# Muennighoff/sgpt

Hardware: AMD Instinct MI355X
Metric: encoded sentences/sec (SGPT-125M, seq_len 128, encode + weighted-mean pool + cosine top-10 chunk loop) (higher is better)
Workload: dtype f16

## Files before the change

### include/sgpt_hip.h

```cpp
#ifndef SGPT_HIP_H
#define SGPT_HIP_H

#include <stddef.h>
#include <stdint.h>

#ifdef __cplusplus
extern "C" {
#endif

#define SGPT_ABI_VERSION 21

typedef int sgpt_status;
#define SGPT_OK 0
#define SGPT_ERR_INVALID (-1)
#define SGPT_ERR_HIP (-2)
#define SGPT_ERR_MISSING (-3)
#define SGPT_ERR_OOM (-4)
#define SGPT_ERR_COMM (-6)
#define SGPT_ERR_RANGE (-5)

typedef struct sgpt_ctx sgpt_ctx;
typedef struct sgpt_model sgpt_model;

enum { SGPT_F32 = 0, SGPT_BF16 = 1, SGPT_FP8W = 2, SGPT_F16 = 3, SGPT_FP8M = 4 };
enum { SGPT_ARCH_GPTNEO = 0, SGPT_ARCH_GPTJ = 1, SGPT_ARCH_BLOOM = 2, SGPT_ARCH_BERT = 3, SGPT_ARCH_LLAMA = 4 };
enum { SGPT_POOL_WEIGHTEDMEAN = 0, SGPT_POOL_MEAN = 1, SGPT_POOL_LASTTOKEN = 2, SGPT_POOL_LEARNTMEAN = 3,
       SGPT_POOL_CLS = 4 };
enum { SGPT_COS = 0, SGPT_DOT = 1, SGPT_NEG_L2 = 2 };

typedef struct {
    int32_t arch;
    int32_t n_layers;
    int32_t d_model;
    int32_t n_heads;
    int32_t d_ffn;
    int32_t vocab;
    int32_t max_pos;
    int32_t window;
    float ln_eps;
    float attn_scale;
    int32_t compute_dtype;
    const uint8_t* layer_is_local;
    int32_t rotary_dim;
    int32_t qk_split;
    int32_t split_weights;
    int32_t n_kv_heads;
} sgpt_model_desc;

typedef struct {
    const char* name;
    const float* ptr;
    int64_t numel;
} sgpt_tensor_view;

int sgpt_abi_version(void);
sgpt_status sgpt_ctx_create(int hip_device, sgpt_ctx** out);
void sgpt_ctx_destroy(sgpt_ctx* ctx);
const char* sgpt_last_error(const sgpt_ctx* ctx);

sgpt_status sgpt_model_load(sgpt_ctx* ctx, const sgpt_model_desc* desc,
                            const sgpt_tensor_view* tensors, size_t n_tensors, sgpt_model** out);
void sgpt_model_free(sgpt_model* model);

sgpt_status sgpt_model_calibrate_begin(sgpt_model* model);
sgpt_status sgpt_model_calibrate_end(sgpt_model* model, float margin, float* scales_out);
sgpt_status sgpt_model_set_act_scales(sgpt_model* model, const float* scales, int32_t n_scales);

sgpt_status sgpt_encode(sgpt_model* model, const int32_t* ids, const int32_t* pos,
                        const int32_t* seq_off, const int32_t* seq_len, const int32_t* pad_left,
                        int32_t B, int32_t T_pad, int32_t max_alloc_len,
                        int32_t pool_mode, int32_t n_layers_run, int32_t apply_final_ln,
                        int32_t normalize, float* out, float* hidden_out, void* stream);

sgpt_status sgpt_encode_layers(sgpt_model* model, const int32_t* ids, const int32_t* pos,
                               const int32_t* seq_off, const int32_t* seq_len, const int32_t* pad_left,
                               int32_t B, int32_t T_pad, int32_t max_alloc_len, int32_t pool_mode,
                               int32_t normalize, float* out_layers, float* out_mean, void* stream);

sgpt_status sgpt_model_set_pool_weights(sgpt_model* model, const float* weights, int32_t n);

sgpt_status sgpt_lm_logprobs(sgpt_model* model, const float* hidden, const int32_t* row_idx, const int32_t* targets,
                             int32_t n, float* out_logprob, int32_t* out_greedy, void* stream);

sgpt_status sgpt_pool(sgpt_ctx* ctx, const void* hidden, int32_t hidden_dtype, const int32_t* mask,
                      int32_t B, int32_t S, int32_t d, int32_t pool_mode, float* out, void* stream);
sgpt_status sgpt_pool_learnt(sgpt_ctx* ctx, const void* hidden, int32_t hidden_dtype, const int32_t* mask,
                             int32_t B, int32_t S, int32_t d, const float* pos_weights, float* out, void* stream);

sgpt_status sgpt_l2_normalize(sgpt_ctx* ctx, const float* in, int64_t n, int32_t d,
                              void* out, int32_t out_dtype, void* stream);

sgpt_status sgpt_pairwise_scores(sgpt_ctx* ctx, const float* a, const float* b, int64_t n, int32_t d, int32_t cosine,
                                 float* out, void* stream);

sgpt_status sgpt_f32_to_16(sgpt_ctx* ctx, const float* in, int64_t numel, void* out, int32_t out_dtype, void* stream);
sgpt_status sgpt_f32_to_bf16(sgpt_ctx* ctx, const float* in, int64_t numel, void* out, void* stream);

sgpt_status sgpt_model_range_check(sgpt_model* model, int32_t* flagged, int32_t reset, void* stream);
sgpt_status sgpt_model_range_adapt(sgpt_model* model, int32_t* n_raised, void* stream);
sgpt_status sgpt_model_get_range_shifts(sgpt_model* model, int32_t* shifts, int32_t n);
sgpt_status sgpt_model_set_range_shifts(sgpt_model* model, const int32_t* shifts, int32_t n);
sgpt_status sgpt_range_check(sgpt_ctx* ctx, int32_t* flagged, int32_t reset, void* stream);

#define SGPT_PREC_CLASSES 5
enum { SGPT_PC_LN1 = 0, SGPT_PC_ATT = 1, SGPT_PC_CTX = 2, SGPT_PC_LN2 = 3, SGPT_PC_H = 4 };
sgpt_status sgpt_model_set_precision(sgpt_model* model, const int32_t* plan, int32_t n);
sgpt_status sgpt_model_get_precision(sgpt_model* model, int32_t* plan, int32_t n);
sgpt_status sgpt_model_release_split_weights(sgpt_model* model, int64_t* bytes_freed);
sgpt_status sgpt_model_precision_probe_begin(sgpt_model* model);
sgpt_status sgpt_model_precision_probe_end(sgpt_model* model, float* crest_out );
sgpt_status sgpt_row_crest(sgpt_ctx* ctx, const void* x, int32_t dtype, int64_t n, int32_t d, int64_t ld, float* crest_out,
                           void* stream);
sgpt_status sgpt_split16(sgpt_ctx* ctx, const float* in, int64_t n, int32_t d, int32_t layout, void* out, int32_t out_dtype,
                         void* stream);
sgpt_status sgpt_linear_split(sgpt_ctx* ctx, int32_t dtype, int32_t epi, const void* A, const void* W, const float* bias,
                              void* out, int64_t ldo, int64_t lo_delta, int64_t hi2_delta, int32_t M, int32_t N, int32_t K,
                              void* stream);

uint64_t sgpt_ctx_generation(const sgpt_ctx* ctx);
sgpt_status sgpt_ctx_reserve(sgpt_ctx* ctx, size_t encode_bytes, size_t score_bytes);

sgpt_status sgpt_fp8_quantize_rows(sgpt_ctx* ctx, const float* w, int64_t rows, int64_t cols,
                                   uint8_t* codes, float* scale, void* stream);
sgpt_status sgpt_fp8_dequantize_rows(sgpt_ctx* ctx, const uint8_t* codes, const float* scale, int64_t rows,
                                     int64_t cols, void* out, int32_t out_dtype, void* stream);

sgpt_status sgpt_scores(sgpt_ctx* ctx, const void* a, const void* b, int32_t dtype,
                        int64_t na, int64_t nb, int32_t d, float* out, int64_t ldo, void* stream);

sgpt_status sgpt_score_topk(sgpt_ctx* ctx, const void* q, const void* corpus, int32_t dtype,
                            int32_t nq, int64_t N, int32_t d, int32_t k, int64_t idx_base,
                            float* run_val, int64_t* run_idx, int32_t n_run, int32_t* n_out,
                            void* stream);

sgpt_status sgpt_score_topk_q8(sgpt_ctx* ctx, const void* q, const uint8_t* codes, const float* scale, int32_t nq, int64_t N, int32_t d,
                               int32_t k, int64_t idx_base, float* run_val, int64_t* run_idx, int32_t n_run, int32_t* n_out,
                               void* stream);

sgpt_status sgpt_pack_sign_bits(sgpt_ctx* ctx, const float* x, int64_t n, int32_t d, const float* center ,
                                uint8_t* bits, int64_t ldb, void* stream);

sgpt_status sgpt_score_topk_bits(sgpt_ctx* ctx, const float* q, const uint8_t* bits, int64_t ldb, int32_t nq, int64_t N, int32_t d,
                                 int32_t k, int32_t kp, int32_t mode, const uint8_t* codes, const float* scale, int64_t idx_base,
                                 float* run_val, int64_t* run_idx, int32_t n_run, int32_t* n_out, void* stream);

sgpt_status sgpt_u8_col_minmax(sgpt_ctx* ctx, const float* x, int64_t n, int32_t d, int32_t accumulate, float* col_min, float* col_max,
                               void* stream);
sgpt_status sgpt_u8_quantize_rows(sgpt_ctx* ctx, const float* x, int64_t n, int32_t d, int32_t ld, const float* start, const float* step,
                                  uint8_t* codes, void* stream);
sgpt_status sgpt_u8_dequantize_rows(sgpt_ctx* ctx, const uint8_t* codes, int64_t n, int32_t ld, const float* start, const float* step,
                                    void* out, int32_t out_dtype, void* stream);

sgpt_status sgpt_u8_prepare_queries(sgpt_ctx* ctx, const float* q, const float* start, const float* step, int32_t nq, int32_t d, int32_t ld,
                                    void* qpad, float* qscale, float* qbias, void* stream);

sgpt_status sgpt_score_topk_u8(sgpt_ctx* ctx, const float* q, const uint8_t* codes, const float* start, const float* step, int32_t nq,
                               int64_t N, int32_t d, int32_t ld, int32_t k, int64_t idx_base, float* run_val, int64_t* run_idx,
                               int32_t n_run, int32_t* n_out, void* stream);

sgpt_status sgpt_u8_rescore(sgpt_ctx* ctx, const float* q, const uint8_t* codes, const float* start, const float* step, int32_t nq, int64_t N,
                            int32_t d, int32_t ld, const int64_t* idx, int64_t ld_idx, int32_t m, int64_t idx_base, float* out_val,
                            int64_t* out_idx, void* stream);

sgpt_status sgpt_score_topk_bits_u8(sgpt_ctx* ctx, const float* q, const float* center , const uint8_t* bits, int64_t ldb,
                                    const uint8_t* codes, const float* start, const float* step, int32_t ld, int32_t nq, int64_t N, int32_t d,
                                    int32_t k, int32_t kp, int64_t idx_base, float* run_val, int64_t* run_idx, int32_t n_run, int32_t* n_out,
                                    void* stream);

sgpt_status sgpt_score_overflow_count(sgpt_ctx* ctx, int32_t* n_chunks, int32_t* n_overflowed, void* stream);

sgpt_status sgpt_score_topk_refined(sgpt_ctx* ctx, const float* q, const float* corpus32, const void* corpus16, int32_t dtype16,
                                    int32_t nq, int64_t N, int32_t d, int32_t k, int64_t idx_base, float margin,
                                    float* run_val, int64_t* run_idx, int32_t n_run, int32_t* n_out, int32_t* fallback_flag_out,
                                    void* stream);

sgpt_status sgpt_topk_merge(sgpt_ctx* ctx, const float* val, const int64_t* idx, int32_t nq,
                            int32_t m, int32_t k, const int64_t* exclude_idx,
                            float* out_val, int64_t* out_idx, void* stream);

#define SGPT_COMM_ID_BYTES 128
sgpt_status sgpt_comm_unique_id(uint8_t* id );
sgpt_status sgpt_comm_init(sgpt_ctx* ctx, const uint8_t* id, int32_t rank, int32_t world);
sgpt_status sgpt_comm_destroy(sgpt_ctx* ctx);
int32_t sgpt_comm_world(const sgpt_ctx* ctx);
int32_t sgpt_comm_rank(const sgpt_ctx* ctx);
sgpt_status sgpt_allgather_rows(sgpt_ctx* ctx, const void* local, const int64_t* counts, int64_t row_bytes, void* out,
                                void* stream);
sgpt_status sgpt_allgather_rows_padded(sgpt_ctx* ctx, const void* local, const int64_t* counts, int64_t row_bytes, void* out,
                                       void* stream);
sgpt_status sgpt_exchange_topk(sgpt_ctx* ctx, const float* val, const int64_t* idx, int32_t nq, int32_t k, int32_t k_out,
                               const int64_t* exclude_idx, float* out_val, int64_t* out_idx, void* stream);
sgpt_status sgpt_fold_gathered_topk(sgpt_ctx* ctx, const float* gathered_val, const int64_t* gathered_idx, int32_t world,
                                    int32_t nq, int32_t k, int32_t k_out, const int64_t* exclude_idx, float* out_val,
                                    int64_t* out_idx, void* stream);

sgpt_status sgpt_topk(sgpt_ctx* ctx, const float* scores, int32_t nq, int64_t n, int64_t ld,
                      int32_t k, int64_t idx_base, float* out_val, int64_t* out_idx, void* stream);

#define SGPT_EVAL_MAX_CUTS 16
sgpt_status sgpt_eval_ranked(sgpt_ctx* ctx, const int64_t* idx, const float* val, int32_t nq, int32_t K,
                             const int32_t* qrel_off, const int64_t* qrel_pos, const int32_t* qrel_rel,
                             const int32_t* ideal_rel, const int32_t* k_values, int32_t nk, int32_t check_order,
                             int32_t* out_hits, int32_t* out_first, float* out_dcg, float* out_idcg, float* out_sp,
                             int32_t* out_R, void* stream);

#define SGPT_EVAL_MAX_GROUP 1024
sgpt_status sgpt_eval_groups(sgpt_ctx* ctx, const float* emb, int32_t n_rows, int32_t d, int32_t mode, const float* scores_in,
                             int32_t G, const int32_t* grp_off, int32_t n_cand, int32_t max_group, const int32_t* q_row,
                             const int32_t* cand_row, const int32_t* cand_rel, const int32_t* R_extra,
                             const int32_t* ideal_off, const int32_t* ideal_rel, int32_t n_ideal, float* out_scores,
                             int32_t* out_order, int32_t* out_hits1, int32_t* out_hits5, int32_t* out_first, int32_t* out_R, float* out_sp,
                             float* out_dcg, float* out_idcg, void* stream);

#define SGPT_EVAL_MAX_PAIRS (1 << 24)
sgpt_status sgpt_eval_pairs(sgpt_ctx* ctx, const float* score, const int32_t* label, int32_t n, int32_t check_nan,
                            int32_t* out_rank2, int64_t* out_n_pos, int64_t* out_n_used, double* out_ap_num, void* stream);

sgpt_status sgpt_linear(sgpt_ctx* ctx, int32_t dtype, int32_t epi, int32_t out_dtype, const void* A, const void* W,
                        const float* bias, const float* resid, void* out, int32_t M, int32_t N, int32_t K, void* stream);

sgpt_status sgpt_linear_query(sgpt_ctx* ctx, int32_t dtype, int32_t epi, const void* A, const float* x, const float* ln_gamma,
                              const float* ln_beta, float ln_eps, const void* W, const float* bias, const float* resid, void* out,
                              void* out_vt, int32_t n_split, int32_t M, int32_t N, int32_t K, void* stream);

sgpt_status sgpt_linear_qkv(sgpt_ctx* ctx, int32_t dtype, const void* A, const void* W, void* out, void* out_vt, int32_t n_split,
                            int32_t M, int32_t N, int32_t K, void* stream);

sgpt_status sgpt_attention(sgpt_ctx* ctx, int32_t dtype, const void* q, const void* k, const void* v, int64_t ldq, int64_t ldvt,
                           void* out, int64_t ldo, const int32_t* seq_off, int32_t B, int32_t T, int32_t H, int32_t dh,
                           int32_t window, float scale, const float* alibi, int32_t max_alloc_len, int32_t out_fp8,
                           float out_scale, int32_t* range_flag, int32_t x3, int64_t qk_lo_delta, int64_t v_lo_delta,
                           int64_t ctx_lo_delta, int64_t ctx_hi2_delta, void* stream);

sgpt_status sgpt_attention_ex(sgpt_ctx* ctx, int32_t dtype, const void* q, const void* k, const void* v, int64_t ldq, int64_t ldvt,
                              void* out, int64_t ldo, const int32_t* seq_off, int32_t B, int32_t T, int32_t H, int32_t dh,
                              int32_t window, float scale, const float* alibi, int32_t max_alloc_len, int32_t out_fp8,
                              float out_scale, int32_t* range_flag, int32_t x3, int64_t qk_lo_delta, int64_t v_lo_delta,
                              int64_t ctx_lo_delta, int64_t ctx_hi2_delta, int32_t causal, const int32_t* seq_len, void* stream);

sgpt_status sgpt_attention_gqa(sgpt_ctx* ctx, int32_t dtype, const void* q, const void* k, const void* v, int64_t ldq, int64_t ldvt,
                               void* out, int64_t ldo, const int32_t* seq_off, int32_t B, int32_t T, int32_t H, int32_t n_kv_heads,
                               int32_t dh, int32_t window, float scale, const float* alibi, int32_t max_alloc_len, int32_t out_fp8,
                               float out_scale, int32_t* range_flag, int32_t x3, int64_t qk_lo_delta, int64_t v_lo_delta,
                               int64_t ctx_lo_delta, int64_t ctx_hi2_delta, void* stream);

sgpt_status sgpt_embed(sgpt_ctx* ctx, const int32_t* ids, const int32_t* pos, const float* wte, const float* wpe, int32_t T,
                       int32_t d, int32_t vocab, int32_t max_pos, float* out, void* stream);
sgpt_status sgpt_layernorm(sgpt_ctx* ctx, const float* x, const float* gamma, const float* beta, int32_t T, int32_t d, float eps,
                           void* out, int32_t out_dtype, float out_mul, int32_t split, void* stream);
sgpt_status sgpt_layernorm_writeback(sgpt_ctx* ctx, float* x, const float* gamma, const float* beta, int32_t T, int32_t d, float eps,
                                     void* out16, int32_t out_dtype, void* stream);
sgpt_status sgpt_rmsnorm(sgpt_ctx* ctx, const float* x, const float* gamma, int32_t T, int32_t d, float eps, void* out, int32_t out_dtype,
                         void* stream);
sgpt_status sgpt_swiglu(sgpt_ctx* ctx, const void* gu, int32_t dtype, int32_t T, int32_t ffn, void* out, void* stream);
sgpt_status sgpt_rope_half(sgpt_ctx* ctx, void* buf, int32_t dtype, int64_t ld, int64_t k_off, const int32_t* pos, const float* sin_t,
                           const float* cos_t, int32_t T, int32_t H, int32_t H_kv, int32_t head_dim, int32_t max_pos, void* stream);
sgpt_status sgpt_qknorm_rope_half(sgpt_ctx* ctx, void* buf, int32_t dtype, int64_t ld, int64_t k_off, const int32_t* pos,
                                  const float* sin_t, const float* cos_t, int32_t T, int32_t H, int32_t H_kv, int32_t head_dim,
                                  int32_t max_pos, const float* q_gamma, const float* k_gamma, float eps, void* stream);
sgpt_status sgpt_lnf_pool_ex(sgpt_ctx* ctx, const float* x, const float* gamma, const float* beta, const int32_t* seq_off,
                             const int32_t* seq_len, const int32_t* pad_left, int32_t B, int32_t d, float eps, int32_t apply_ln,
                             int32_t mode, int32_t normalize, const float* pos_weights, int32_t n_weights, float* out,
                             int32_t* nonfinite_flag, int32_t norm_kind, void* stream);
sgpt_status sgpt_lnf_pool(sgpt_ctx* ctx, const float* x, const float* gamma, const float* beta, const int32_t* seq_off,
                          const int32_t* seq_len, const int32_t* pad_left, int32_t B, int32_t d, float eps, int32_t apply_ln,
                          int32_t mode, int32_t normalize, const float* pos_weights, int32_t n_weights, float* out,
                          int32_t* nonfinite_flag, void* stream);
sgpt_status sgpt_rope(sgpt_ctx* ctx, void* buf, int32_t dtype, int64_t ld, int64_t k_off, const int32_t* pos, const float* sin,
                      const float* cos, int32_t T, int32_t H, int32_t head_dim, int32_t rotary_dim, int32_t max_pos, void* stream);
sgpt_status sgpt_logprob_rows(sgpt_ctx* ctx, const float* logits, int64_t ld, int32_t V, const int32_t* targets, int32_t n,
                              float* out_logprob, int32_t* out_greedy, void* stream);

sgpt_status sgpt_layernorm_fp8(sgpt_ctx* ctx, const float* x, const float* gamma, const float* beta, int32_t T, int32_t d,
                               float eps, uint8_t* codes, float* row_scale, void* stream);
sgpt_status sgpt_linear_fp8(sgpt_ctx* ctx, int32_t epi, int32_t out_dtype, const uint8_t* A, const float* a_scale,
                            float a_scalar, const uint8_t* W, const float* w_scale, const float* bias, const float* resid,
                            void* out, float out_scale, int32_t M, int32_t N, int32_t K, void* stream);

sgpt_status sgpt_prof_enable(sgpt_ctx* ctx, int32_t on);
sgpt_status sgpt_prof_read(sgpt_ctx* ctx, int64_t* launches, double* ms, double* flops, int32_t reset);

int32_t sgpt_ctx_set_gemm_cu_cap(sgpt_ctx* ctx, int32_t n);
int32_t sgpt_ctx_set_low_latency(sgpt_ctx* ctx, int32_t on);
int32_t sgpt_ctx_set_tile_policy(sgpt_ctx* ctx, int32_t policy);
int32_t sgpt_ctx_set_query_tile(sgpt_ctx* ctx, int32_t k);

sgpt_status sgpt_bench_gemm(sgpt_ctx* ctx, int32_t dtype, int32_t epi, int32_t out_dtype,
                            int32_t M, int32_t N, int32_t K, int32_t iters, float* ms_out);

#ifdef __cplusplus
}
#endif
#endif
```

### sgpt_amd/_lib.py

```python
import ctypes as C
import os

HERE = os.path.dirname(os.path.abspath(__file__))
LIB_PATH = os.environ.get("SGPT_HIP_LIB") or os.path.join(HERE, "lib", "libsgpt_hip.so")

SGPT_F32, SGPT_BF16, SGPT_FP8W, SGPT_F16, SGPT_FP8M = 0, 1, 2, 3, 4
SGPT_ABI_VERSION = 21
SGPT_PREC_CLASSES = 5
PC_LN1, PC_ATT, PC_CTX, PC_LN2, PC_H = 0, 1, 2, 3, 4
SGPT_ERR_RANGE = -5
SGPT_ERR_COMM = -6
SGPT_COMM_ID_BYTES = 128
SGPT_EVAL_MAX_CUTS = 16
SGPT_EVAL_MAX_GROUP = 1024
SGPT_EVAL_MAX_PAIRS = 1 << 24
SGPT_COS, SGPT_DOT, SGPT_NEG_L2 = 0, 1, 2
SGPT_ARCH_GPTNEO, SGPT_ARCH_GPTJ, SGPT_ARCH_BLOOM, SGPT_ARCH_BERT, SGPT_ARCH_LLAMA = 0, 1, 2, 3, 4
POOL_MODES = {"weightedmean": 0, "mean": 1, "lasttoken": 2, "learntmean": 3, "cls": 4}
EPI_BIAS_GELU_ERF = 9


class ModelDesc(C.Structure):
    _fields_ = [("arch", C.c_int32), ("n_layers", C.c_int32), ("d_model", C.c_int32), ("n_heads", C.c_int32),
                ("d_ffn", C.c_int32), ("vocab", C.c_int32), ("max_pos", C.c_int32), ("window", C.c_int32),
                ("ln_eps", C.c_float), ("attn_scale", C.c_float), ("compute_dtype", C.c_int32),
                ("layer_is_local", C.POINTER(C.c_uint8)), ("rotary_dim", C.c_int32), ("qk_split", C.c_int32),
                ("split_weights", C.c_int32), ("n_kv_heads", C.c_int32)]


class TensorView(C.Structure):
    _fields_ = [("name", C.c_char_p), ("ptr", C.c_void_p), ("numel", C.c_int64)]


SIGNATURES = {
    "sgpt_abi_version": (C.c_int, []),
    "sgpt_ctx_create": (C.c_int, [C.c_int, C.POINTER(C.c_void_p)]),
    "sgpt_ctx_destroy": (None, [C.c_void_p]),
    "sgpt_last_error": (C.c_char_p, [C.c_void_p]),
    "sgpt_model_load": (C.c_int, [C.c_void_p, C.POINTER(ModelDesc), C.POINTER(TensorView), C.c_size_t,
                                  C.POINTER(C.c_void_p)]),
    "sgpt_model_free": (None, [C.c_void_p]),
    "sgpt_encode": (C.c_int, [C.c_void_p, C.c_void_p, C.c_void_p, C.c_void_p, C.c_void_p, C.c_void_p,
                              C.c_int32, C.c_int32, C.c_int32, C.c_int32, C.c_int32, C.c_int32, C.c_int32,
                              C.c_void_p, C.c_void_p, C.c_void_p]),
    "sgpt_encode_layers": (C.c_int, [C.c_void_p, C.c_void_p, C.c_void_p, C.c_void_p, C.c_void_p, C.c_void_p,
                                     C.c_int32, C.c_int32, C.c_int32, C.c_int32, C.c_int32, C.c_void_p, C.c_void_p,
                                     C.c_void_p]),
    "sgpt_model_set_pool_weights": (C.c_int, [C.c_void_p, C.c_void_p, C.c_int32]),
    "sgpt_pool_learnt": (C.c_int, [C.c_void_p, C.c_void_p, C.c_int32, C.c_void_p, C.c_int32, C.c_int32, C.c_int32,
                                   C.c_void_p, C.c_void_p, C.c_void_p]),
    "sgpt_fp8_quantize_rows": (C.c_int, [C.c_void_p, C.c_void_p, C.c_int64, C.c_int64, C.c_void_p, C.c_void_p,
                                         C.c_void_p]),
    "sgpt_fp8_dequantize_rows": (C.c_int, [C.c_void_p, C.c_void_p, C.c_void_p, C.c_int64, C.c_int64, C.c_void_p,
                                           C.c_int32, C.c_void_p]),
    "sgpt_lm_logprobs": (C.c_int, [C.c_void_p, C.c_void_p, C.c_void_p, C.c_void_p, C.c_int32, C.c_void_p, C.c_void_p,
                                   C.c_void_p]),
    "sgpt_pool": (C.c_int, [C.c_void_p, C.c_void_p, C.c_int32, C.c_void_p, C.c_int32, C.c_int32, C.c_int32,
                            C.c_int32, C.c_void_p, C.c_void_p]),
    "sgpt_l2_normalize": (C.c_int, [C.c_void_p, C.c_void_p, C.c_int64, C.c_int32, C.c_void_p, C.c_int32, C.c_void_p]),
    "sgpt_pairwise_scores": (C.c_int, [C.c_void_p, C.c_void_p, C.c_void_p, C.c_int64, C.c_int32, C.c_int32, C.c_void_p, C.c_void_p]),
    "sgpt_f32_to_bf16": (C.c_int, [C.c_void_p, C.c_void_p, C.c_int64, C.c_void_p, C.c_void_p]),
    "sgpt_f32_to_16": (C.c_int, [C.c_void_p, C.c_void_p, C.c_int64, C.c_void_p, C.c_int32, C.c_void_p]),
    "sgpt_range_check": (C.c_int, [C.c_void_p, C.POINTER(C.c_int32), C.c_int32, C.c_void_p]),
    "sgpt_ctx_generation": (C.c_uint64, [C.c_void_p]),
    "sgpt_ctx_reserve": (C.c_int, [C.c_void_p, C.c_size_t, C.c_size_t]),
    "sgpt_scores": (C.c_int, [C.c_void_p, C.c_void_p, C.c_void_p, C.c_int32, C.c_int64, C.c_int64, C.c_int32,
                              C.c_void_p, C.c_int64, C.c_void_p]),
    "sgpt_score_topk": (C.c_int, [C.c_void_p, C.c_void_p, C.c_void_p, C.c_int32, C.c_int32, C.c_int64, C.c_int32,
                                  C.c_int32, C.c_int64, C.c_void_p, C.c_void_p, C.c_int32, C.POINTER(C.c_int32),
                                  C.c_void_p]),
    "sgpt_score_topk_q8": (C.c_int, [C.c_void_p, C.c_void_p, C.c_void_p, C.c_void_p, C.c_int32, C.c_int64, C.c_int32,
                                     C.c_int32, C.c_int64, C.c_void_p, C.c_void_p, C.c_int32, C.POINTER(C.c_int32),
                                     C.c_void_p]),
    "sgpt_score_topk_u8": (C.c_int, [C.c_void_p, C.c_void_p, C.c_void_p, C.c_void_p, C.c_void_p, C.c_int32, C.c_int64, C.c_int32, C.c_int32,
                                     C.c_int32, C.c_int64, C.c_void_p, C.c_void_p, C.c_int32, C.POINTER(C.c_int32), C.c_void_p]),
    "sgpt_u8_col_minmax": (C.c_int, [C.c_void_p, C.c_void_p, C.c_int64, C.c_int32, C.c_int32, C.c_void_p, C.c_void_p, C.c_void_p]),
    "sgpt_u8_quantize_rows": (C.c_int, [C.c_void_p, C.c_void_p, C.c_int64, C.c_int32, C.c_int32, C.c_void_p, C.c_void_p, C.c_void_p,
                                        C.c_void_p]),
    "sgpt_u8_dequantize_rows": (C.c_int, [C.c_void_p, C.c_void_p, C.c_int64, C.c_int32, C.c_void_p, C.c_void_p, C.c_void_p, C.c_int32,
                                          C.c_void_p]),
    "sgpt_u8_prepare_queries": (C.c_int, [C.c_void_p, C.c_void_p, C.c_void_p, C.c_void_p, C.c_int32, C.c_int32, C.c_int32, C.c_void_p,
                                          C.c_void_p, C.c_void_p, C.c_void_p]),
    "sgpt_pack_sign_bits": (C.c_int, [C.c_void_p, C.c_void_p, C.c_int64, C.c_int32, C.c_void_p, C.c_void_p, C.c_int64, C.c_void_p]),
    "sgpt_score_topk_bits": (C.c_int, [C.c_void_p, C.c_void_p, C.c_void_p, C.c_int64, C.c_int32, C.c_int64, C.c_int32, C.c_int32,
                                       C.c_int32, C.c_int32, C.c_void_p, C.c_void_p, C.c_int64, C.c_void_p, C.c_void_p, C.c_int32,
                                       C.POINTER(C.c_int32), C.c_void_p]),
    "sgpt_u8_rescore": (C.c_int, [C.c_void_p, C.c_void_p, C.c_void_p, C.c_void_p, C.c_void_p, C.c_int32, C.c_int64, C.c_int32, C.c_int32,
                                  C.c_void_p, C.c_int64, C.c_int32, C.c_int64, C.c_void_p, C.c_void_p, C.c_void_p]),
    "sgpt_score_topk_bits_u8": (C.c_int, [C.c_void_p, C.c_void_p, C.c_void_p, C.c_void_p, C.c_int64, C.c_void_p, C.c_void_p, C.c_void_p,
                                          C.c_int32, C.c_int32, C.c_int64, C.c_int32, C.c_int32, C.c_int32, C.c_int64, C.c_void_p,
                                          C.c_void_p, C.c_int32, C.POINTER(C.c_int32), C.c_void_p]),
    "sgpt_score_overflow_count": (C.c_int, [C.c_void_p, C.POINTER(C.c_int32), C.POINTER(C.c_int32), C.c_void_p]),
    "sgpt_score_topk_refined": (C.c_int, [C.c_void_p, C.c_void_p, C.c_void_p, C.c_void_p, C.c_int32, C.c_int32, C.c_int64, C.c_int32,
                                           C.c_int32, C.c_int64, C.c_float, C.c_void_p, C.c_void_p, C.c_int32, C.c_void_p, C.c_void_p,
                                           C.c_void_p]),
    "sgpt_topk_merge": (C.c_int, [C.c_void_p, C.c_void_p, C.c_void_p, C.c_int32, C.c_int32, C.c_int32, C.c_void_p,
                                  C.c_void_p, C.c_void_p, C.c_void_p]),
    "sgpt_topk": (C.c_int, [C.c_void_p, C.c_void_p, C.c_int32, C.c_int64, C.c_int64, C.c_int32, C.c_int64,
                            C.c_void_p, C.c_void_p, C.c_void_p]),
    "sgpt_eval_ranked": (C.c_int, [C.c_void_p, C.c_void_p, C.c_void_p, C.c_int32, C.c_int32, C.c_void_p, C.c_void_p, C.c_void_p,
                                   C.c_void_p, C.POINTER(C.c_int32), C.c_int32, C.c_int32, C.c_void_p, C.c_void_p, C.c_void_p,
                                   C.c_void_p, C.c_void_p, C.c_void_p, C.c_void_p]),
    "sgpt_eval_groups": (C.c_int, [C.c_void_p, C.c_void_p, C.c_int32, C.c_int32, C.c_int32, C.c_void_p, C.c_int32, C.c_void_p, C.c_int32,
                                   C.c_int32, C.c_void_p, C.c_void_p, C.c_void_p, C.c_void_p, C.c_void_p, C.c_void_p, C.c_int32,
                                   C.c_void_p, C.c_void_p, C.c_void_p, C.c_void_p, C.c_void_p, C.c_void_p, C.c_void_p, C.c_void_p,
                                   C.c_void_p, C.c_void_p]),
    "sgpt_eval_pairs": (C.c_int, [C.c_void_p, C.c_void_p, C.c_void_p, C.c_int32, C.c_int32, C.c_void_p, C.c_void_p, C.c_void_p,
                                  C.c_void_p, C.c_void_p]),
    "sgpt_linear": (C.c_int, [C.c_void_p, C.c_int32, C.c_int32, C.c_int32, C.c_void_p, C.c_void_p, C.c_void_p, C.c_void_p,
                              C.c_void_p, C.c_int32, C.c_int32, C.c_int32, C.c_void_p]),
    "sgpt_linear_query": (C.c_int, [C.c_void_p, C.c_int32, C.c_int32, C.c_void_p, C.c_void_p, C.c_void_p, C.c_void_p, C.c_float, C.c_void_p,
                                    C.c_void_p, C.c_void_p, C.c_void_p, C.c_void_p, C.c_int32, C.c_int32, C.c_int32, C.c_int32, C.c_void_p]),
    "sgpt_linear_qkv": (C.c_int, [C.c_void_p, C.c_int32, C.c_void_p, C.c_void_p, C.c_void_p, C.c_void_p, C.c_int32, C.c_int32, C.c_int32,
                                  C.c_int32, C.c_void_p]),
    "sgpt_model_calibrate_begin": (C.c_int, [C.c_void_p]),
    "sgpt_model_calibrate_end": (C.c_int, [C.c_void_p, C.c_float, C.c_void_p]),
    "sgpt_model_set_act_scales": (C.c_int, [C.c_void_p, C.c_void_p, C.c_int32]),
    "sgpt_layernorm_fp8": (C.c_int, [C.c_void_p, C.c_void_p, C.c_void_p, C.c_void_p, C.c_int32, C.c_int32, C.c_float, C.c_void_p,
                                     C.c_void_p, C.c_void_p]),
    "sgpt_linear_fp8": (C.c_int, [C.c_void_p, C.c_int32, C.c_int32, C.c_void_p, C.c_void_p, C.c_float, C.c_void_p, C.c_void_p,
                                  C.c_void_p, C.c_void_p, C.c_void_p, C.c_float, C.c_int32, C.c_int32, C.c_int32, C.c_void_p]),
    "sgpt_comm_unique_id": (C.c_int, [C.c_void_p]),
    "sgpt_comm_init": (C.c_int, [C.c_void_p, C.c_void_p, C.c_int32, C.c_int32]),
    "sgpt_comm_destroy": (C.c_int, [C.c_void_p]),
    "sgpt_comm_world": (C.c_int32, [C.c_void_p]),
    "sgpt_comm_rank": (C.c_int32, [C.c_void_p]),
    "sgpt_allgather_rows": (C.c_int, [C.c_void_p, C.c_void_p, C.c_void_p, C.c_int64, C.c_void_p, C.c_void_p]),
    "sgpt_allgather_rows_padded": (C.c_int, [C.c_void_p, C.c_void_p, C.c_void_p, C.c_int64, C.c_void_p, C.c_void_p]),
    "sgpt_exchange_topk": (C.c_int, [C.c_void_p, C.c_void_p, C.c_void_p, C.c_int32, C.c_int32, C.c_int32, C.c_void_p,
                                     C.c_void_p, C.c_void_p, C.c_void_p]),
    "sgpt_fold_gathered_topk": (C.c_int, [C.c_void_p, C.c_void_p, C.c_void_p, C.c_int32, C.c_int32, C.c_int32, C.c_int32,
                                          C.c_void_p, C.c_void_p, C.c_void_p, C.c_void_p]),
    "sgpt_ctx_set_low_latency": (C.c_int32, [C.c_void_p, C.c_int32]),
    "sgpt_ctx_set_tile_policy": (C.c_int32, [C.c_void_p, C.c_int32]),
    "sgpt_ctx_set_gemm_cu_cap": (C.c_int32, [C.c_void_p, C.c_int32]),
    "sgpt_ctx_set_query_tile": (C.c_int32, [C.c_void_p, C.c_int32]),
    "sgpt_model_range_check": (C.c_int, [C.c_void_p, C.POINTER(C.c_int32), C.c_int32, C.c_void_p]),
    "sgpt_model_range_adapt": (C.c_int, [C.c_void_p, C.POINTER(C.c_int32), C.c_void_p]),
    "sgpt_model_get_range_shifts": (C.c_int, [C.c_void_p, C.c_void_p, C.c_int32]),
    "sgpt_model_set_range_shifts": (C.c_int, [C.c_void_p, C.c_void_p, C.c_int32]),
    "sgpt_model_set_precision": (C.c_int, [C.c_void_p, C.c_void_p, C.c_int32]),
    "sgpt_model_get_precision": (C.c_int, [C.c_void_p, C.c_void_p, C.c_int32]),
    "sgpt_model_release_split_weights": (C.c_int, [C.c_void_p, C.c_void_p]),
    "sgpt_model_precision_probe_begin": (C.c_int, [C.c_void_p]),
    "sgpt_model_precision_probe_end": (C.c_int, [C.c_void_p, C.c_void_p]),
    "sgpt_row_crest": (C.c_int, [C.c_void_p, C.c_void_p, C.c_int32, C.c_int64, C.c_int32, C.c_int64, C.POINTER(C.c_float), C.c_void_p]),
    "sgpt_split16": (C.c_int, [C.c_void_p, C.c_void_p, C.c_int64, C.c_int32, C.c_int32, C.c_void_p, C.c_int32, C.c_void_p]),
    "sgpt_linear_split": (C.c_int, [C.c_void_p, C.c_int32, C.c_int32, C.c_void_p, C.c_void_p, C.c_void_p, C.c_void_p,
                                    C.c_int64, C.c_int64, C.c_int64, C.c_int32, C.c_int32, C.c_int32, C.c_void_p]),
    "sgpt_attention": (C.c_int, [C.c_void_p, C.c_int32, C.c_void_p, C.c_void_p, C.c_void_p, C.c_int64, C.c_int64,
                                 C.c_void_p, C.c_int64, C.c_void_p, C.c_int32, C.c_int32, C.c_int32, C.c_int32,
                                 C.c_int32, C.c_float, C.c_void_p, C.c_int32, C.c_int32,
                                 C.c_float, C.c_void_p, C.c_int32, C.c_int64, C.c_int64,
                                 C.c_int64, C.c_int64, C.c_void_p]),
    "sgpt_attention_ex": (C.c_int, [C.c_void_p, C.c_int32, C.c_void_p, C.c_void_p, C.c_void_p, C.c_int64, C.c_int64,
                                    C.c_void_p, C.c_int64, C.c_void_p, C.c_int32, C.c_int32, C.c_int32, C.c_int32,
                                    C.c_int32, C.c_float, C.c_void_p, C.c_int32, C.c_int32,
                                    C.c_float, C.c_void_p, C.c_int32, C.c_int64, C.c_int64,
                                    C.c_int64, C.c_int64, C.c_int32, C.c_void_p, C.c_void_p]),
    "sgpt_attention_gqa": (C.c_int, [C.c_void_p, C.c_int32, C.c_void_p, C.c_void_p, C.c_void_p, C.c_int64, C.c_int64,
                                     C.c_void_p, C.c_int64, C.c_void_p, C.c_int32, C.c_int32, C.c_int32, C.c_int32, C.c_int32,
                                     C.c_int32, C.c_float, C.c_void_p, C.c_int32, C.c_int32,
                                     C.c_float, C.c_void_p, C.c_int32, C.c_int64, C.c_int64,
                                     C.c_int64, C.c_int64, C.c_void_p]),
    "sgpt_rmsnorm": (C.c_int, [C.c_void_p, C.c_void_p, C.c_void_p, C.c_int32, C.c_int32, C.c_float, C.c_void_p, C.c_int32, C.c_void_p]),
    "sgpt_swiglu": (C.c_int, [C.c_void_p, C.c_void_p, C.c_int32, C.c_int32, C.c_int32, C.c_void_p, C.c_void_p]),
    "sgpt_rope_half": (C.c_int, [C.c_void_p, C.c_void_p, C.c_int32, C.c_int64, C.c_int64, C.c_void_p, C.c_void_p, C.c_void_p,
                                 C.c_int32, C.c_int32, C.c_int32, C.c_int32, C.c_int32, C.c_void_p]),
    "sgpt_qknorm_rope_half": (C.c_int, [C.c_void_p, C.c_void_p, C.c_int32, C.c_int64, C.c_int64, C.c_void_p, C.c_void_p, C.c_void_p,
                                        C.c_int32, C.c_int32, C.c_int32, C.c_int32, C.c_int32, C.c_void_p, C.c_void_p, C.c_float,
                                        C.c_void_p]),
    "sgpt_lnf_pool_ex": (C.c_int, [C.c_void_p, C.c_void_p, C.c_void_p, C.c_void_p, C.c_void_p, C.c_void_p, C.c_void_p, C.c_int32,
                                   C.c_int32, C.c_float, C.c_int32, C.c_int32, C.c_int32, C.c_void_p, C.c_int32, C.c_void_p,
                                   C.c_void_p, C.c_int32, C.c_void_p]),
    "sgpt_layernorm_writeback": (C.c_int, [C.c_void_p, C.c_void_p, C.c_void_p, C.c_void_p, C.c_int32, C.c_int32, C.c_float, C.c_void_p,
                                           C.c_int32, C.c_void_p]),
    "sgpt_embed": (C.c_int, [C.c_void_p, C.c_void_p, C.c_void_p, C.c_void_p, C.c_void_p, C.c_int32, C.c_int32, C.c_int32, C.c_int32,
                             C.c_void_p, C.c_void_p]),
    "sgpt_layernorm": (C.c_int, [C.c_void_p, C.c_void_p, C.c_void_p, C.c_void_p, C.c_int32, C.c_int32, C.c_float, C.c_void_p,
                                 C.c_int32, C.c_float, C.c_int32, C.c_void_p]),
    "sgpt_lnf_pool": (C.c_int, [C.c_void_p, C.c_void_p, C.c_void_p, C.c_void_p, C.c_void_p, C.c_void_p, C.c_void_p, C.c_int32,
                                C.c_int32, C.c_float, C.c_int32, C.c_int32, C.c_int32, C.c_void_p, C.c_int32, C.c_void_p,
                                C.c_void_p, C.c_void_p]),
    "sgpt_rope": (C.c_int, [C.c_void_p, C.c_void_p, C.c_int32, C.c_int64, C.c_int64, C.c_void_p, C.c_void_p, C.c_void_p,
                            C.c_int32, C.c_int32, C.c_int32, C.c_int32, C.c_int32, C.c_void_p]),
    "sgpt_logprob_rows": (C.c_int, [C.c_void_p, C.c_void_p, C.c_int64, C.c_int32, C.c_void_p, C.c_int32, C.c_void_p, C.c_void_p,
                                    C.c_void_p]),
    "sgpt_bench_gemm": (C.c_int, [C.c_void_p, C.c_int32, C.c_int32, C.c_int32, C.c_int32, C.c_int32, C.c_int32,
                                  C.c_int32, C.POINTER(C.c_float)]),
    "sgpt_prof_enable": (C.c_int, [C.c_void_p, C.c_int32]),
    "sgpt_prof_read": (C.c_int, [C.c_void_p, C.POINTER(C.c_int64), C.POINTER(C.c_double), C.POINTER(C.c_double),
                                 C.c_int32]),
}

_lib = None


class SgptHipError(RuntimeError):
    pass


class SgptRangeError(SgptHipError):
    """dtype='f16': a weight is outside the IEEE-half range, or an activation class is beyond every power-of-two range
    shift (use dtype='bf16'); dtype='fp8mfma': an e4m3 code saturated (re-calibrate)."""

EXPERIMENT_SIGNATURES = {
    "sgpt_exp_set_gemm_skew": (C.c_int32, [C.c_int32]),
    "sgpt_exp_set_gemm_w": (C.c_int32, [C.c_int32]),
}


def load():
    global _lib
    if _lib is not None:
        return _lib
    if not os.path.exists(LIB_PATH):
        raise SgptHipError(f"{LIB_PATH} is missing: build it with `python -m sgpt_amd.build` "
                           "(hipcc --offload-arch=gfx950); there is no CPU/PyTorch fallback")
    lib = C.CDLL(LIB_PATH)
    for name, (res, args) in SIGNATURES.items():
        fn = getattr(lib, name)
        fn.restype = res
        fn.argtypes = args
    for name, (res, args) in EXPERIMENT_SIGNATURES.items():
        if hasattr(lib, name):
            fn = getattr(lib, name)
            fn.restype = res
            fn.argtypes = args
    if lib.sgpt_abi_version() != SGPT_ABI_VERSION:
        raise SgptHipError("libsgpt_hip.so ABI version mismatch: rebuild with `python -m sgpt_amd.build --force`")
    _lib = lib
    return lib


def check(ctx_handle, status, what=""):
    if status == 0:
        return
    msg = load().sgpt_last_error(ctx_handle)
    msg = msg.decode() if msg else ""
    if status == -1:
        raise ValueError(f"{what}: {msg}")
    if status == SGPT_ERR_RANGE:
        raise SgptRangeError(f"{what}: {msg}")
    raise SgptHipError(f"{what}: status {status}: {msg}")
```

### sgpt_amd/csrc/common.h

```cpp
#pragma once
#include <hip/hip_runtime.h>
#include <stdint.h>

typedef uint16_t bf16_t;
struct f16_t { uint16_t bits; };
typedef __attribute__((ext_vector_type(8))) __bf16 bf16x8;
typedef __attribute__((ext_vector_type(8))) _Float16 f16x8;
typedef __attribute__((ext_vector_type(4))) float f32x4;
typedef __attribute__((ext_vector_type(16))) float f32x16;

constexpr int DT_F32 = 0, DT_BF16 = 1, DT_FP8W = 2, DT_F16 = 3;
__host__ __device__ constexpr bool dt_is16(int dt) { return dt == DT_BF16 || dt == DT_F16; }

#define WAVE 64

typedef uint2 __attribute__((may_alias)) uint2_a;
typedef uint4 __attribute__((may_alias)) uint4_a;
typedef float4 __attribute__((may_alias)) float4_a;

__device__ __forceinline__ float bf16_to_f32(bf16_t v) { return __uint_as_float(((uint32_t)v) << 16); }

typedef __attribute__((ext_vector_type(2))) __bf16 bf16x2_t;
typedef __attribute__((ext_vector_type(2))) float f32x2_t;
__device__ __forceinline__ uint32_t pack_bf16x2(float lo, float hi) {
// ... 98 lines not shown
#pragma unroll
    for (int o = 32; o > 0; o >>= 1) v += __shfl_xor(v, o, 64);
    return v;
}
template <int CTRL> __device__ __forceinline__ float dpp_mov(float v) {
    return __uint_as_float((unsigned)__builtin_amdgcn_update_dpp(0, (int)__float_as_uint(v), CTRL, 0xf, 0xf, false));
}
__device__ __forceinline__ float wave_sum_valu(float v) {
    { const auto r = __builtin_amdgcn_permlane32_swap(__float_as_uint(v), __float_as_uint(v), false, false);
      v = __uint_as_float(r[0]) + __uint_as_float(r[1]); }
    { const auto r = __builtin_amdgcn_permlane16_swap(__float_as_uint(v), __float_as_uint(v), false, false);
      v = __uint_as_float(r[0]) + __uint_as_float(r[1]); }
    v += dpp_mov<0x128>(v);
    v += dpp_mov<0x1B>(dpp_mov<0x141>(v));
    v += dpp_mov<0x4E>(v);
    v += dpp_mov<0xB1>(v);
    return v;
}
template <int R>
__device__ __forceinline__ void wave_sum_valu_multi(float (&v)[R]) {
#pragma unroll
    for (int u = 0; u < R; ++u) {
        const auto r = __builtin_amdgcn_permlane32_swap(__float_as_uint(v[u]), __float_as_uint(v[u]), false, false);
        v[u] = __uint_as_float(r[0]) + __uint_as_float(r[1]);
    }
#pragma unroll
    for (int u = 0; u < R; ++u) {
        const auto r = __builtin_amdgcn_permlane16_swap(__float_as_uint(v[u]), __float_as_uint(v[u]), false, false);
        v[u] = __uint_as_float(r[0]) + __uint_as_float(r[1]);
    }
#pragma unroll
    for (int u = 0; u < R; ++u) v[u] += dpp_mov<0x128>(v[u]);
#pragma unroll
    for (int u = 0; u < R; ++u) v[u] += dpp_mov<0x1B>(dpp_mov<0x141>(v[u]));
#pragma unroll
    for (int u = 0; u < R; ++u) v[u] += dpp_mov<0x4E>(v[u]);
#pragma unroll
    for (int u = 0; u < R; ++u) v[u] += dpp_mov<0xB1>(v[u]);
}
__device__ __forceinline__ float wave_max(float v) {
#pragma unroll
    for (int o = 32; o > 0; o >>= 1) v = fmaxf(v, __shfl_xor(v, o, 64));
    return v;
}

__device__ __forceinline__ float gelu_new(float u) {
    const float c = 0.7978845608028654f;
    float t = c * (u + 0.044715f * u * u * u);
    return 0.5f * u * (1.0f + tanhf(t));
}

__device__ __forceinline__ float gelu_erf(float u) { return 0.5f * u * (1.0f + erff(u * 0.70710678118654752f)); }

__device__ __forceinline__ float gelu_new_fast(float u) {
    const float k0 = -2.0f * 0.7978845608028654f * 1.4426950408889634f;
    const float k1 = k0 * 0.044715f;
    const float z = u * __builtin_fmaf(u * u, k1, k0);
    return u * __builtin_amdgcn_rcpf(1.0f + __builtin_amdgcn_exp2f(z));
}

__device__ __forceinline__ float gelu_new_fast_scaled(float u, float inv) {
    const float k0 = -2.0f * 0.7978845608028654f * 1.4426950408889634f;
    const float k1 = k0 * 0.044715f;
    const float z = u * __builtin_fmaf(u * u, k1, k0);
    return u * __builtin_amdgcn_rcpf(__builtin_fmaf(__builtin_amdgcn_exp2f(z), inv, inv));
}

__device__ __forceinline__ bool cand_room(const int* cnt, int cap) {
    return __hip_atomic_load(cnt, __ATOMIC_RELAXED, __HIP_MEMORY_SCOPE_AGENT) <= cap;
}

inline int device_cu_count() {
    static const int ncu = [] {
        int dev = 0, n = 256;
        (void)hipGetDevice(&dev);
        (void)hipDeviceGetAttribute(&n, hipDeviceAttributeMultiprocessorCount, dev);
        return n;
    }();
    return ncu;
}

enum GemmEpi {
    EPI_STORE = 0,
    EPI_BIAS_GELU = 1,
    EPI_BIAS_RESID = 2,
    EPI_SCORE = 3,
    EPI_VT = 4,
    EPI_NONE = 5,
    EPI_SCORE_FILTER = 6,
    EPI_SCORE_TOP2 = 8,
    EPI_BIAS_GELU_ERF = 9,
    EPI_QKV = 7,
};

__host__ __device__ constexpr bool epi_is_gelu(int epi) { return epi == EPI_BIAS_GELU || epi == EPI_BIAS_GELU_ERF; }

struct GemmArgs {
    const void* A;
    const void* W;
    void* out;
    const float* bias;
    const float* resid;
    int M, N, K;
    long lda, ldw, ldo;
    int m_valid;
    int skew;
    int gm, gn;
    int balanced;
    const int* pred;
    const float* thr;
    long thr_ld;
    float* cand_val;
    long long* cand_idx;
    int* cand_cnt;
    int cand_cap;
    long idx_base;
    long long* dbg;
    int* range_flag;
    unsigned* range_amax;
    float in_mul, out_mul, out_mul2;
    int k_algo;
    int kgroups;
    int force256;
    int cu_cap;
    long lo_delta, hi2_delta, lo_delta2;
    void* out2;
    long ldo2;
    int n_split;
    int n_valid;
    const float* a_scale;
    const float* w_scale;
    float a_scalar;
    float out_scale;
};

void launch_gemm(int dtype, int epi, int out_dtype, const GemmArgs& a, hipStream_t s);
constexpr int QGEMM_MAX_ROWS = 4096;
struct QGemmArgs {
    GemmArgs g;
    const float* x;
    const float* ln_g;
    const float* ln_b;
    float eps, ln_mul;
    int group;
    int tile;
};
bool qgemm_shape_ok(int M, int N, int K, int epi, int n_split);
bool qgemm_ln_ok(int M, int N, int d, int epi, int n_split);
bool launch_qgemm(int dtype, int epi, int out_dtype, const QGemmArgs& a, hipStream_t s);

bool gemm_qkv_one_launch(int M, int n_split, bool force256);
bool gemm_score_tail_foldable(int M, long N, int K);
bool gemm_qkv_bulk(int M, int N, int K, int n_split, bool force256);
#ifdef SGPT_EXPERIMENTS
int set_gemm_skew(int cycles);
int set_gemm_use_w(int on);
#endif
bool gemm_fp8_shape_ok(int M, int N, int K);
void launch_gemm_fp8(int epi, int out_dtype, const GemmArgs& a, hipStream_t s);
struct Score8Args {
    GemmArgs g;
    const float* scale;
    long scale_stride;
};
bool score64q8_shape_ok(int M, long N, int K, const void* codes, long ldw);
void launch_score64q8(int epi, const Score8Args& a, hipStream_t s);
struct ScoreU8Args {
    GemmArgs g;
    const float* qscale;
    const float* qbias;
};
bool score64u8_shape_ok(int M, long N, int K, const void* codes, long ldw);
void launch_score64u8(int epi, const ScoreU8Args& a, hipStream_t s);
void launch_u8_prepare_queries(const float* q, const float* start, const float* step, int nq, int d, int ld, void* qpad, float* qscale,
                               float* qbias, hipStream_t s);
void launch_u8_col_minmax(const float* x, long n, int d, int accumulate, float* mn, float* mx, hipStream_t s);
void launch_u8_quant_rows(const float* x, long n, int d, int ld, const float* start, const float* step, uint8_t* codes, hipStream_t s);
void launch_u8_dequant_rows(const uint8_t* codes, long n, int ld, const float* start, const float* step, void* out, int out_dtype,
                            hipStream_t s);
void launch_u8_rescore_prepare(const float* q, const float* start, const float* step, int nq, int d, int ld, float* qs, float* qbias,
                               hipStream_t s);
void launch_u8_rescore(const float* qs, const float* qbias, const uint8_t* codes, int ld, const int64_t* idx, long ld_idx, int nq, int m,
                       long idx_base, long n_docs, float* out_val, int64_t* out_idx, long ld_out, hipStream_t s);
void launch_scorebits(int epi, const GemmArgs& g, int d, int qw, long ldb, hipStream_t s, bool spread = false);
void launch_gemm256w(int dtype, int epi, const GemmArgs& a, hipStream_t s, bool deep_a);

struct AttnArgs {
    const void* q;
    const void* k;
    const void* v;
    void* ctx;
    const int* seq_off;
    int B, H, dh;
    long ldq, ldvt, ldo;
    int window;
    float scale;
    int max_alloc_len;
    const float* alibi;
    int dtype;
    int out_fp8;
    float out_scale;
    int* range_flag;
    int x3;
    long qk_lo_delta, v_lo_delta, ctx_lo_delta, ctx_hi2_delta;
    int noncausal;
    const int* seq_len;
    int kv_group = 1;
};
inline bool attn_x3_supported(int dh) { return dh == 64 || dh == 128; }
void launch_attn_bf16(const AttnArgs& a, hipStream_t s);
void launch_attn_f32(const AttnArgs& a, hipStream_t s);

void launch_embed(const int* ids, const int* pos, const float* wte, const float* wpe, float* x, int T, int d, int vocab,
                  int max_pos, hipStream_t s);
void launch_layernorm(const float* x, const float* g, const float* b, void* out, int out_dtype, int T, int d,
                      float eps, hipStream_t s, float out_mul = 1.0f);
void launch_layernorm_writeback(float* x, const float* g, const float* b, void* out16, int out_dtype, int T, int d, float eps,
                                int* range_flag, hipStream_t s);
void launch_layernorm_split(const float* x, const float* g, const float* b, void* out, int out_dtype, int T, int d,
                            float eps, hipStream_t s, float out_mul);
void launch_rmsnorm(const float* x, const float* g, void* out, int out_dtype, int T, int d, float eps, int* range_flag, hipStream_t s);
void launch_swiglu(const void* gu, void* h, int dtype, int T, int ffn, int* range_flag, hipStream_t s);
void launch_pack_split_rows(const float* src, long rows, long cols, void* dst, int out_dtype, hipStream_t s);
void launch_crest16(const void* in, int T, int cols, long ld, int dtype, unsigned* out_bits, hipStream_t s);
void launch_split16_rows(const float* in, long n, int d, int layout, void* out, int out_dtype, hipStream_t s);
void launch_layernorm_q8(const float* x, const float* g, const float* b, void* q, float* scale, int T, int d, float eps, hipStream_t s);
void launch_absmax16(const void* in, long numel, int dtype, unsigned* out_bits, hipStream_t s);
void launch_lnf_pool(const float* x, const float* g, const float* b, const int* seq_off, const int* seq_len,
                     const int* pad_left, int B, int d, float eps, int apply_ln, int mode, int normalize,
                     const float* pos_weights, int pos_weights_n, float* out, hipStream_t s,
                     int* nonfinite_flag = nullptr,
                     int norm_kind = 0);
void launch_pool(const void* hidden, int dtype, const int* mask, int B, int S, int d, int mode,
                 const float* pos_weights, float* out, hipStream_t s);
void launch_fp8_quant_rows(const float* w, long rows, long cols, void* q, float* scale, hipStream_t s);
void launch_fp8_dequant_rows(const void* q, const float* scale, long rows, long cols, void* out, int out_dtype,
                             hipStream_t s);
void launch_l2norm(const float* in, long n, int d, void* out, int out_dtype, hipStream_t s);
void launch_pack_sign_bits(const float* x, long n, int d, const float* center, uint8_t* bits, long ldb, hipStream_t s);
void launch_pairwise(const float* a, const float* b, long n, int d, bool cosine, float* out, hipStream_t s);
void launch_gather_rows(const float* src, const int* row_idx, int n, int d, float* dst, hipStream_t s);
void launch_logprob_rows(const float* logits, long ld, int V, const int* targets, int n, float* out_lp, int* out_arg,
                         hipStream_t s);
void launch_mean_over_axis0(const float* in, int n0, long n, float* out, hipStream_t s);
void launch_f32_to_16(const float* in, long numel, void* out, int out_dtype, hipStream_t s);
void launch_absmax(const float* in, long numel, unsigned* out_bits, hipStream_t s);
void launch_fill_f32(float* p, long n, float v, hipStream_t s);
void launch_rope(void* qk, int dtype, long ld, long k_off, const int* pos, const float* sin_t, const float* cos_t, int T,
                 int H, int dh, int rotary_dim, int max_pos, hipStream_t s);
void launch_rope_half(void* qk, int dtype, long ld, long k_off, const int* pos, const float* sin_t, const float* cos_t, int T,
                      int H, int H_kv, int dh, int max_pos, hipStream_t s);
void launch_qknorm_rope_half(void* qk, int dtype, long ld, long k_off, const int* pos, const float* sin_t, const float* cos_t,
                             const float* q_g, const float* k_g, float eps, int T, int H, int H_kv, int dh, int max_pos, int* range_flag,
                             hipStream_t s);
void launch_qkv_deinterleave(const float* src, float* dst, int H, int dh, long row_len, hipStream_t s);
void launch_fill_rand(void* p, long n, int dtype, unsigned seed, float scale, hipStream_t s);

void launch_topk_select(const float* scores, long ld, long n, long idx_base, const float* prev_val,
                        const int64_t* prev_idx, int n_prev, long prev_ld, int nq, int k, int nan_to_m1,
                        const int64_t* exclude_idx, float* out_val, int64_t* out_idx, hipStream_t s,
                        const int* pred = nullptr, float* thr_out = nullptr,
                        int gather_k = 0);
void launch_rescore(const float* q, const float* corpus, const int64_t* idx, long ld_idx, int nq, int m, int d, long idx_base,
                    long n_docs, float* out_val, int64_t* out_idx, long ld_out, hipStream_t s);
void launch_rescore_bits(int mode, const float* q, const uint8_t* bits, long ldb, const uint8_t* codes, long ld8, const float* scale,
                         const float* val1, const int64_t* idx, long ld_idx, int nq, int m, int d, long idx_base, long n_docs,
                         float* out_val, int64_t* out_idx, long ld_out, hipStream_t s);
void launch_refine_check(const float* v16, int k, int kp, float margin, int nq, int* flag, hipStream_t s);
void launch_list_append(const float* in_val, const int64_t* in_idx, long ld_in, int n_run, int nq, float* out_val, int64_t* out_idx,
                        long ld_out, int col0, hipStream_t s);
void launch_score_prep(const void* q, void* qpad, long q_bytes, long qpad_bytes, int* counters, long n_counters, long long* idx_list,
                       long n_idx, hipStream_t s);
void launch_thr_below(const float* list, int k, int nq, float* thr, hipStream_t s);
void launch_cand_merge(const float* run_val, const int64_t* run_idx, const float* cand_val, const int64_t* cand_idx,
                       int* cand_cnt, int cap, int nq, int k, float* out_val, int64_t* out_idx, int* overflow,
                       hipStream_t s, float* thr_io = nullptr);
```

### sgpt_amd/csrc/ctx.h

```cpp
#pragma once
#include <hip/hip_runtime.h>

#include <string>
#include <utility>
#include <vector>

struct sgpt_ctx {
    int device = 0;
    std::string err;
    void* ws = nullptr; size_t ws_bytes = 0;
    void* ws2 = nullptr; size_t ws2_bytes = 0;
    void* ws3 = nullptr; size_t ws3_bytes = 0;
    void* ws4 = nullptr; size_t ws4_bytes = 0;
    void* ws5 = nullptr; size_t ws5_bytes = 0;
    void* ws6 = nullptr; size_t ws6_bytes = 0;
    size_t filt_flag_off = 0; int filt_chunks = 0;
    void* comm = nullptr;
    int comm_rank = 0, comm_world = 0;
    uint64_t generation = 0;
    int* range_flag = nullptr;
    int kgroups = 1;
    int force256 = 0;
    int no_qpath = 0;
    int cu_cap = 0;
    int qtile = 0;
    bool prof = false;
    std::vector<std::pair<hipEvent_t, hipEvent_t>> ev_pool;
    size_t ev_used = 0;
    std::vector<double> ev_flops;
    int64_t prof_launches = 0; double prof_ms = 0, prof_flops = 0;
};
```

### sgpt_amd/csrc/ctx.hip

```cpp
#include "host.h"

namespace sgpt_host {

sgpt_status ensure(sgpt_ctx* c, void** p, size_t* have, size_t need) {
    if (*have >= need) return SGPT_OK;
    if (*p) { HIPC(c, hipDeviceSynchronize()); HIPC(c, hipFree(*p)); *p = nullptr; *have = 0; }
    need = align_up(need + (need >> 3), 1 << 20);
    if (hipMalloc(p, need) != hipSuccess) { *p = nullptr; return fail(c, SGPT_ERR_OOM, "hipMalloc workspace failed"); }
    HIPC(c, hipMemset(*p, 0, need));
    *have = need;
    c->generation++;
    return SGPT_OK;
}

void gemm(sgpt_ctx* c, int dtype, int epi, int out_dtype, const GemmArgs& a0, hipStream_t s) {
    Prof p(c, s, 2.0 * (double)a0.m_valid * a0.N * (a0.k_algo > 0 ? a0.k_algo : a0.K));
    GemmArgs a = a0;
    a.kgroups = c->kgroups; a.force256 = c->force256; a.cu_cap = c->cu_cap;
    launch_gemm(dtype, epi, out_dtype, a, s);
}

bool qgemm(sgpt_ctx* c, int dtype, int epi, int out_dtype, const QGemmArgs& a, hipStream_t s) {
    Prof p(c, s, 2.0 * (double)a.g.m_valid * a.g.N * a.g.K);
    return launch_qgemm(dtype, epi, out_dtype, a, s);
}

}

extern "C" {

int sgpt_abi_version(void) { return SGPT_ABI_VERSION; }

sgpt_status sgpt_ctx_create(int hip_device, sgpt_ctx** out) {
    if (!out) return SGPT_ERR_INVALID;
    *out = nullptr;
    int n = 0;
    if (hipGetDeviceCount(&n) != hipSuccess || hip_device < 0 || hip_device >= n) return SGPT_ERR_HIP;
    if (hipSetDevice(hip_device) != hipSuccess) return SGPT_ERR_HIP;
    sgpt_ctx* c = new sgpt_ctx();
    c->device = hip_device;
    if (hipMalloc((void**)&c->range_flag, 256) != hipSuccess || hipMemset(c->range_flag, 0, 256) != hipSuccess) {
        delete c;
        return SGPT_ERR_OOM;
    }
    *out = c;
    return SGPT_OK;
}

void sgpt_ctx_destroy(sgpt_ctx* c) {
    if (!c) return;
    (void)hipSetDevice(c->device);
    (void)hipDeviceSynchronize();
    if (c->ws) (void)hipFree(c->ws);
    if (c->ws2) (void)hipFree(c->ws2);
    (void)sgpt_comm_destroy(c);
    if (c->ws3) (void)hipFree(c->ws3);
    if (c->ws4) (void)hipFree(c->ws4);
    if (c->ws5) (void)hipFree(c->ws5);
    if (c->ws6) (void)hipFree(c->ws6);
    if (c->range_flag) (void)hipFree(c->range_flag);
    for (auto& e : c->ev_pool) { (void)hipEventDestroy(e.first); (void)hipEventDestroy(e.second); }
    delete c;
}

const char* sgpt_last_error(const sgpt_ctx* c) { return c ? c->err.c_str() : "null ctx"; }

uint64_t sgpt_ctx_generation(const sgpt_ctx* c) { return c ? c->generation : 0; }

sgpt_status sgpt_ctx_reserve(sgpt_ctx* c, size_t encode_bytes, size_t score_bytes) {
    if (!c) return SGPT_ERR_INVALID;
    HIPC(c, hipSetDevice(c->device));
    sgpt_status st = ensure(c, &c->ws, &c->ws_bytes, encode_bytes);
    if (st != SGPT_OK) return st;
    return ensure(c, &c->ws2, &c->ws2_bytes, score_bytes);
}

sgpt_status sgpt_range_check(sgpt_ctx* c, int32_t* flagged, int32_t reset, void* stream) {
    if (!c || !flagged) return SGPT_ERR_INVALID;
    HIPC(c, hipSetDevice(c->device));
    hipStream_t s = (hipStream_t)stream;
    int h = 0;
    HIPC(c, hipMemcpyAsync(&h, c->range_flag, sizeof(int), hipMemcpyDeviceToHost, s));
    HIPC(c, hipStreamSynchronize(s));
    if (reset && h) HIPC(c, hipMemsetAsync(c->range_flag, 0, sizeof(int), s));
    *flagged = h;
    return SGPT_OK;
}

sgpt_status sgpt_prof_enable(sgpt_ctx* c, int32_t on) {
    if (!c) return SGPT_ERR_INVALID;
    c->prof = on != 0;
    return SGPT_OK;
}

sgpt_status sgpt_prof_read(sgpt_ctx* c, int64_t* launches, double* ms, double* flops, int32_t reset) {
    if (!c) return SGPT_ERR_INVALID;
    HIPC(c, hipSetDevice(c->device));
    HIPC(c, hipDeviceSynchronize());
    for (size_t i = 0; i < c->ev_used; ++i) {
        float t = 0;
        HIPC(c, hipEventElapsedTime(&t, c->ev_pool[i].first, c->ev_pool[i].second));
        c->prof_ms += t;
        c->prof_flops += c->ev_flops[i];
        c->prof_launches++;
    }
    c->ev_used = 0;
    if (launches) *launches = c->prof_launches;
    if (ms) *ms = c->prof_ms;
    if (flops) *flops = c->prof_flops;
    if (reset) { c->prof_launches = 0; c->prof_ms = 0; c->prof_flops = 0; }
    return SGPT_OK;
}

int32_t sgpt_ctx_set_low_latency(sgpt_ctx* c, int32_t on) {
    if (!c) return 0;
    const int old = c->kgroups > 1 ? 1 : 0;
    c->kgroups = on ? 2 : 1;
    return old;
}
int32_t sgpt_ctx_set_gemm_cu_cap(sgpt_ctx* c, int32_t n) {
    if (!c) return 0;
    const int old = c->cu_cap;
    c->cu_cap = n > 0 ? n : 0;
    return old;
}
int32_t sgpt_ctx_set_tile_policy(sgpt_ctx* c, int32_t policy) {
    if (!c) return 0;
    const int old = c->force256 ? 1 : c->no_qpath ? 2 : 0;
    c->force256 = policy == 1 ? 1 : 0;
    c->no_qpath = policy == 2 ? 1 : 0;
    return old;
}
int32_t sgpt_ctx_set_query_tile(sgpt_ctx* c, int32_t k) {
    if (!c || k < 0 || k > 7) return -1;
    const int old = c->qtile;
    c->qtile = k;
    return old;
}
#ifdef SGPT_EXPERIMENTS
int32_t sgpt_exp_set_gemm_skew(int32_t cycles) { return set_gemm_skew(cycles); }
int32_t sgpt_exp_set_gemm_w(int32_t on) { return set_gemm_use_w(on); }
#endif

}
```

### sgpt_amd/csrc/encode.hip

```cpp
#include "host.h"

namespace {

struct Fwd {
    sgpt_model* m; sgpt_ctx* c; hipStream_t s;
    const Family* F;
    const int32_t *pos, *seq_off, *seq_len;
    int B, T, max_alloc;
    int d_q, d_kv;
    int dt;
    int* range_flag;
    bool can_split, any_ln, any_att, any_ctx, any_h, split, fp8, mlp8, qpath, qln;
    float* x;
    void *a, *ctx, *qkv, *vt, *h;
    void* gu;
    void* a8; float* sa;
    long att_lo;
};

GemmArgs proj(const Fwd& f, const void* A, long lda, const void* W, int N, int K, void* out, long ldo, const float* bias,
              const float* resid = nullptr) {
    GemmArgs g{};
    g.M = f.T; g.m_valid = f.T; g.range_flag = f.range_flag;
    g.A = A; g.lda = lda; g.W = W; g.ldw = K; g.N = N; g.K = K; g.out = out; g.ldo = ldo; g.bias = bias; g.resid = resid;
    return g;
}

void split_w(GemmArgs& g, const void* W3, int k, int nblk = 3) { g.W = W3; g.K = nblk * k; g.ldw = 3 * k; g.k_algo = k; }

void proj_qk_vt(const Fwd& f, const GemmArgs& g, int n_qk, int n_v, const void* W3 = nullptr, int p_ln1 = 0) {
    GemmArgs qk = g, v = g;
    if (p_ln1) split_w(qk, W3, g.K, p_ln1 == 3 ? 2 : 3);
    qk.N = n_qk;
    gemm(f.c, f.dt, EPI_STORE, f.dt, qk, f.s);
    if (p_ln1 == 2) split_w(v, (const bf16_t*)W3 + (size_t)n_qk * 3 * g.K, g.K);
    else v.W = (const bf16_t*)g.W + (size_t)n_qk * g.K;
    v.N = n_v; v.out = f.vt; v.ldo = f.T; v.bias = g.bias ? g.bias + n_qk : nullptr;
    gemm(f.c, f.dt, EPI_VT, f.dt, v, f.s);
}

AttnArgs attn_base(const Fwd& f, const LayerW& l, int k_qkv) {
    const sgpt_model_desc& d = f.m->d;
    const int dq = f.d_q;
    AttnArgs at{};
    at.dtype = f.dt;
    at.seq_off = f.seq_off; at.B = f.B; at.H = d.n_heads; at.dh = dq / d.n_heads; at.window = l.is_local ? d.window : 0;
    at.scale = d.attn_scale * pow2f(2 * k_qkv);
    at.max_alloc_len = f.max_alloc; at.ctx = f.ctx; at.ldo = dq; at.alibi = f.m->alibi;
    at.q = f.qkv; at.kv_group = d.n_heads / d.n_kv_heads;
    if (f.vt) { at.k = (bf16_t*)f.qkv + dq; at.v = f.vt; at.ldq = dq + f.d_kv; at.ldvt = f.T; }
    else { at.k = (float*)f.qkv + dq; at.v = (float*)f.qkv + dq + f.d_kv; at.ldq = dq + 2 * f.d_kv; }
    return at;
}

AttnArgs attn_bidir(const Fwd& f, const LayerW& l) {
    AttnArgs at = attn_base(f, l, 0);
    at.noncausal = 1; at.seq_len = f.seq_len;
    return at;
}

sgpt_status block_bert_f32(const Fwd& f, const LayerW& l, int) {
    const sgpt_model_desc& d = f.m->d;
    const int dm = d.d_model, ffn = d.d_ffn, T = f.T;
    gemm(f.c, SGPT_F32, EPI_STORE, SGPT_F32, proj(f, f.x, dm, l.w_qkv, 3 * dm, dm, f.qkv, 3 * dm, l.b_qkv), f.s);
    launch_attn_f32(attn_bidir(f, l), f.s);
    gemm(f.c, SGPT_F32, EPI_BIAS_RESID, SGPT_F32, proj(f, f.ctx, dm, l.w_o, dm, dm, f.x, dm, l.b_o, f.x), f.s);
    launch_layernorm(f.x, l.ln1_g, l.ln1_b, f.x, SGPT_F32, T, dm, d.ln_eps, f.s);
    gemm(f.c, SGPT_F32, EPI_BIAS_GELU_ERF, SGPT_F32, proj(f, f.x, dm, l.w_fc, ffn, dm, f.h, ffn, l.b_fc), f.s);
    gemm(f.c, SGPT_F32, EPI_BIAS_RESID, SGPT_F32, proj(f, f.h, ffn, l.w_proj, dm, ffn, f.x, dm, l.b_proj, f.x), f.s);
    launch_layernorm(f.x, l.ln2_g, l.ln2_b, f.x, SGPT_F32, T, dm, d.ln_eps, f.s);
    return SGPT_OK;
}

sgpt_status block_bert16(const Fwd& f, const LayerW& l, int) {
    const sgpt_model_desc& d = f.m->d;
    const int dm = d.d_model, ffn = d.d_ffn, T = f.T, dt = f.dt;
    GemmArgs q = proj(f, f.a, dm, l.w_qkv, 3 * dm, dm, f.qkv, 2 * dm, l.b_qkv);
    if (gemm_qkv_one_launch(T, 2 * dm, f.c->force256 != 0)) {
        q.n_split = 2 * dm; q.out2 = f.vt; q.ldo2 = T;
        gemm(f.c, dt, EPI_QKV, dt, q, f.s);
    } else proj_qk_vt(f, q, 2 * dm, dm);
    launch_attn_bf16(attn_bidir(f, l), f.s);
    gemm(f.c, dt, EPI_BIAS_RESID, SGPT_F32, proj(f, f.ctx, dm, l.w_o, dm, dm, f.x, dm, l.b_o, f.x), f.s);
    launch_layernorm_writeback(f.x, l.ln1_g, l.ln1_b, f.a, dt, T, dm, d.ln_eps, f.range_flag, f.s);
    gemm(f.c, dt, EPI_BIAS_GELU_ERF, dt, proj(f, f.a, dm, l.w_fc, ffn, dm, f.h, ffn, l.b_fc), f.s);
    gemm(f.c, dt, EPI_BIAS_RESID, SGPT_F32, proj(f, f.h, ffn, l.w_proj, dm, ffn, f.x, dm, l.b_proj, f.x), f.s);
    launch_layernorm_writeback(f.x, l.ln2_g, l.ln2_b, f.a, dt, T, dm, d.ln_eps, f.range_flag, f.s);
    return SGPT_OK;
}


void rope_llama(const Fwd& f, const LayerW& l, int dt, long ld, int dh) {
    const sgpt_model_desc& d = f.m->d;
    if (l.qn_g)
        launch_qknorm_rope_half(f.qkv, dt, ld, f.d_q, f.pos, f.m->rot_sin, f.m->rot_cos, l.qn_g, l.kn_g, d.ln_eps, f.T, d.n_heads, d.n_kv_heads,
                                dh, d.max_pos, f.range_flag, f.s);
    else launch_rope_half(f.qkv, dt, ld, f.d_q, f.pos, f.m->rot_sin, f.m->rot_cos, f.T, d.n_heads, d.n_kv_heads, dh, d.max_pos, f.s);
}
sgpt_status block_llama_f32(const Fwd& f, const LayerW& l, int) {
    const sgpt_model_desc& d = f.m->d;
    const int dm = d.d_model, ffn = d.d_ffn, T = f.T, dq = f.d_q, dh = dq / d.n_heads, dkv = f.d_kv;
    launch_rmsnorm(f.x, l.ln1_g, f.a, SGPT_F32, T, dm, d.ln_eps, nullptr, f.s);
    gemm(f.c, SGPT_F32, EPI_STORE, SGPT_F32, proj(f, f.a, dm, l.w_qkv, dq + 2 * dkv, dm, f.qkv, dq + 2 * dkv, l.b_qkv), f.s);
    rope_llama(f, l, SGPT_F32, dq + 2 * dkv, dh);
    launch_attn_f32(attn_base(f, l, 0), f.s);
    gemm(f.c, SGPT_F32, EPI_BIAS_RESID, SGPT_F32, proj(f, f.ctx, dq, l.w_o, dm, dq, f.x, dm, l.b_o, f.x), f.s);
    launch_rmsnorm(f.x, l.ln2_g, f.a, SGPT_F32, T, dm, d.ln_eps, nullptr, f.s);
    gemm(f.c, SGPT_F32, EPI_STORE, SGPT_F32, proj(f, f.a, dm, l.w_fc, 2 * ffn, dm, f.gu, 2 * ffn, nullptr), f.s);
    launch_swiglu(f.gu, f.h, SGPT_F32, T, ffn, nullptr, f.s);
    gemm(f.c, SGPT_F32, EPI_BIAS_RESID, SGPT_F32, proj(f, f.h, ffn, l.w_proj, dm, ffn, f.x, dm, l.b_proj, f.x), f.s);
    return SGPT_OK;
}

sgpt_status block_llama16(const Fwd& f, const LayerW& l, int) {
    const sgpt_model_desc& d = f.m->d;
    const int dm = d.d_model, ffn = d.d_ffn, T = f.T, dt = f.dt, dq = f.d_q, dh = dq / d.n_heads, dkv = f.d_kv;
    launch_rmsnorm(f.x, l.ln1_g, f.a, dt, T, dm, d.ln_eps, f.range_flag, f.s);
    proj_qk_vt(f, proj(f, f.a, dm, l.w_qkv, dq + dkv, dm, f.qkv, dq + dkv, l.b_qkv), dq + dkv, dkv);
    rope_llama(f, l, dt, dq + dkv, dh);
    launch_attn_bf16(attn_base(f, l, 0), f.s);
    gemm(f.c, dt, EPI_BIAS_RESID, SGPT_F32, proj(f, f.ctx, dq, l.w_o, dm, dq, f.x, dm, l.b_o, f.x), f.s);
    launch_rmsnorm(f.x, l.ln2_g, f.a, dt, T, dm, d.ln_eps, f.range_flag, f.s);
    gemm(f.c, dt, EPI_STORE, dt, proj(f, f.a, dm, l.w_fc, 2 * ffn, dm, f.gu, 2 * ffn, nullptr), f.s);
    launch_swiglu(f.gu, f.h, dt, T, ffn, f.range_flag, f.s);
    gemm(f.c, dt, EPI_BIAS_RESID, SGPT_F32, proj(f, f.h, ffn, l.w_proj, dm, ffn, f.x, dm, l.b_proj, f.x), f.s);
    return SGPT_OK;
}

sgpt_status block_f32(const Fwd& f, const LayerW& l, int) {
    const sgpt_model_desc& d = f.m->d;
    const int dm = d.d_model, ffn = d.d_ffn, T = f.T;
    const bool gptj = d.arch == SGPT_ARCH_GPTJ;
    launch_layernorm(f.x, l.ln1_g, l.ln1_b, f.a, SGPT_F32, T, dm, d.ln_eps, f.s);
    gemm(f.c, SGPT_F32, EPI_STORE, SGPT_F32, proj(f, f.a, dm, l.w_qkv, 3 * dm, dm, f.qkv, 3 * dm, l.b_qkv), f.s);
    if (gptj) launch_rope(f.qkv, SGPT_F32, 3 * dm, dm, f.pos, f.m->rot_sin, f.m->rot_cos, T, d.n_heads, dm / d.n_heads, d.rotary_dim, d.max_pos, f.s);
    launch_attn_f32(attn_base(f, l, 0), f.s);
    gemm(f.c, SGPT_F32, EPI_BIAS_RESID, SGPT_F32, proj(f, f.ctx, dm, l.w_o, dm, dm, f.x, dm, l.b_o, f.x), f.s);
    if (!gptj) launch_layernorm(f.x, l.ln2_g, l.ln2_b, f.a, SGPT_F32, T, dm, d.ln_eps, f.s);
    gemm(f.c, SGPT_F32, EPI_BIAS_GELU, SGPT_F32, proj(f, f.a, dm, l.w_fc, ffn, dm, f.h, ffn, l.b_fc), f.s);
    gemm(f.c, SGPT_F32, EPI_BIAS_RESID, SGPT_F32, proj(f, f.h, ffn, l.w_proj, dm, ffn, f.x, dm, l.b_proj, f.x), f.s);
    return SGPT_OK;
}

sgpt_status block_fp8(const Fwd& f, const LayerW& l, int li) {
    const sgpt_model_desc& d = f.m->d;
    const int dm = d.d_model, ffn = d.d_ffn, T = f.T;
    const bool gptj = d.arch == SGPT_ARCH_GPTJ;
    const float s_h = f.m->act_scale[li], s_c = f.m->act_scale[d.n_layers + li];
    auto launch = [&](int epi, int out_dtype, const GemmArgs& q) { Prof pr(f.c, f.s, 2.0 * T * (double)q.N * q.K); launch_gemm_fp8(epi, out_dtype, q, f.s); };
    launch_layernorm_q8(f.x, l.ln1_g, l.ln1_b, f.a8, f.sa, T, dm, d.ln_eps, f.s);
    GemmArgs qk = proj(f, f.a8, dm, l.w_qkv, 2 * dm, dm, f.qkv, 2 * dm, l.b_qkv);
    qk.a_scale = f.sa; qk.a_scalar = 1.0f; qk.w_scale = l.s_qkv;
    launch(EPI_STORE, f.dt, qk);
    GemmArgs v = proj(f, f.a8, dm, (const uint8_t*)l.w_qkv + (size_t)2 * dm * dm, dm, dm, f.vt, T, l.b_qkv ? l.b_qkv + 2 * dm : nullptr);
    v.a_scale = f.sa; v.a_scalar = 1.0f; v.w_scale = l.s_qkv + 2 * dm;
    launch(EPI_VT, f.dt, v);
    if (gptj) launch_rope(f.qkv, f.dt, 2 * dm, dm, f.pos, f.m->rot_sin, f.m->rot_cos, T, d.n_heads, dm / d.n_heads, d.rotary_dim, d.max_pos, f.s);
    AttnArgs at = attn_base(f, l, 0);
    at.out_fp8 = 1; at.out_scale = s_c; at.range_flag = f.range_flag;
    launch_attn_bf16(at, f.s);
    GemmArgs o = proj(f, f.ctx, dm, l.w_o, dm, dm, f.x, dm, l.b_o, f.x);
    o.a_scalar = s_c; o.w_scale = l.s_o;
    launch(EPI_BIAS_RESID, 0, o);
    if (!gptj) launch_layernorm_q8(f.x, l.ln2_g, l.ln2_b, f.a8, f.sa, T, dm, d.ln_eps, f.s);
    GemmArgs fc = proj(f, f.a8, dm, l.w_fc, ffn, dm, f.h, ffn, l.b_fc);
    fc.a_scale = f.sa; fc.a_scalar = 1.0f; fc.w_scale = l.s_fc; fc.out_scale = s_h;
    launch(EPI_BIAS_GELU, 0, fc);
    GemmArgs p = proj(f, f.h, ffn, l.w_proj, dm, ffn, f.x, dm, l.b_proj, f.x);
    p.a_scalar = s_h; p.w_scale = l.s_proj;
    launch(EPI_BIAS_RESID, 0, p);
    return SGPT_OK;
}

void block_ln(const Fwd& f, QGemmArgs& q, const float* g, const float* b, int k, bool split, unsigned* crest) {
    const int dm = f.m->d.d_model;
    const float eps = f.m->d.ln_eps;
    q.eps = eps;
    if (f.qln) { q.x = f.x; q.ln_g = g; q.ln_b = b; q.ln_mul = pow2f(-k); return; }
    if (split) launch_layernorm_split(f.x, g, b, f.a, f.dt, f.T, dm, eps, f.s, pow2f(-k));
    else launch_layernorm(f.x, g, b, f.a, f.dt, f.T, dm, eps, f.s, pow2f(-k));
    if (crest) launch_crest16(f.a, f.T, dm, q.g.lda, f.dt, crest, f.s);
}

sgpt_status launch16(const Fwd& f, int epi, int out_dtype, const QGemmArgs& q, const char* what) {
    if (!f.qpath) gemm(f.c, f.dt, epi, out_dtype, q.g, f.s);
    else if (!qgemm(f.c, f.dt, epi, out_dtype, q, f.s)) return fail(f.c, SGPT_ERR_INVALID, std::string("query path: ") + what + " not served");
    return SGPT_OK;
}

sgpt_status block_16(const Fwd& f, const LayerW& l, int li) {
    sgpt_model* m = f.m; sgpt_ctx* c = f.c; hipStream_t s = f.s;
    const int dm = m->d.d_model, ffn = m->d.d_ffn, T = f.T, dt = f.dt;
    const bool gptj = m->d.arch == SGPT_ARCH_GPTJ;
    const bool f16m = dt == SGPT_F16;
    const int* sh = &m->shift[(size_t)li * RS_N];
    const int k_ln1 = f16m ? sh[RS_LN1] : 0, k_qkv = f16m ? sh[RS_QKV] : 0, k_h = f16m ? sh[RS_H] : 0;
    const int k_ln2 = f16m ? (gptj ? sh[RS_LN1] : sh[RS_LN2]) : 0;
    unsigned* slots = m->range_dev + 1 + (size_t)li * RS_N;
    const int* pc = &m->prec[(size_t)li * PC_N];
    const int p_ln1 = f.can_split ? pc[PC_LN1] : 0;
    const bool p_att = f.can_split && pc[PC_ATT] != 0, p_ctx = f.can_split && pc[PC_CTX] != 0, p_h = f.can_split && pc[PC_H] != 0;
    const bool p_ln2 = f.can_split && pc[PC_LN2] != 0 && (!gptj || p_ln1 != 0);
    unsigned* crest = (m->probing && m->crest_dev) ? m->crest_dev + (size_t)li * RS_N : nullptr;
    const long lda1 = p_ln1 ? 3 * dm : dm, lda2 = gptj ? lda1 : (p_ln2 ? 3 * dm : dm), ldc = p_ctx ? 3 * dm : dm, ldh = p_h ? 3 * ffn : ffn;
    sgpt_status st;
    {
        QGemmArgs q{};
        q.g = proj(f, f.a, lda1, l.w_qkv, 3 * dm, dm, f.qkv, 2 * dm, l.b_qkv);
        q.g.in_mul = pow2f(k_ln1); q.g.out_mul = q.g.out_mul2 = pow2f(-k_qkv); q.g.range_amax = f16m ? slots + RS_QKV : nullptr;
        q.g.lo_delta = q.g.lo_delta2 = p_att ? f.att_lo : 0;
        block_ln(f, q, l.ln1_g, l.ln1_b, k_ln1, p_ln1 != 0, crest ? crest + RS_LN1 : nullptr);
        if (f.qpath || ((p_ln1 == 0 || p_ln1 == 2) && gemm_qkv_one_launch(T, 2 * dm, c->force256 != 0)) ||
            (p_ln1 == 0 && !p_att && l.b_qkv == nullptr && gemm_qkv_bulk(T, 3 * dm, dm, 2 * dm, c->force256 != 0))) {
            if (p_ln1 == 2) split_w(q.g, l.w_qkv3, dm);
            q.g.n_split = 2 * dm; q.g.out2 = f.vt; q.g.ldo2 = T;
            if ((st = launch16(f, EPI_QKV, dt, q, "QKV projection")) != SGPT_OK) return st;
        } else {
            proj_qk_vt(f, q.g, 2 * dm, dm, l.w_qkv3, p_ln1);
        }
    }
    if (gptj) launch_rope(f.qkv, dt, 2 * dm, dm, f.pos, m->rot_sin, m->rot_cos, T, m->d.n_heads, dm / m->d.n_heads, m->d.rotary_dim, m->d.max_pos, s);
    AttnArgs at = attn_base(f, l, k_qkv);
    at.x3 = p_att ? 1 : 0; at.qk_lo_delta = f.att_lo; at.v_lo_delta = f.att_lo;
    at.ldo = ldc; at.ctx_lo_delta = p_ctx ? dm : 0; at.ctx_hi2_delta = p_ctx ? 2 * dm : 0;
    launch_attn_bf16(at, s);
    if (crest) launch_crest16(f.ctx, T, dm, ldc, dt, crest + RS_QKV, s);
    if (m->calibrating)
        launch_absmax16(f.ctx, (long)T * dm, dt, m->h_amax + m->d.n_layers + li, s);
    {
        QGemmArgs q{};
        q.g = proj(f, f.ctx, ldc, l.w_o, dm, dm, f.x, dm, l.b_o, f.x);
        if (p_ctx) split_w(q.g, l.w_o3, dm);
        q.g.in_mul = pow2f(k_qkv);
        if ((st = launch16(f, EPI_BIAS_RESID, SGPT_F32, q, "out-projection")) != SGPT_OK) return st;
    }
    {
        QGemmArgs q{};
        q.g = proj(f, f.a, lda2, l.w_fc, ffn, dm, f.h, ldh, l.b_fc);
        if (p_ln2) split_w(q.g, l.w_fc3, dm);
        if (p_h) { q.g.lo_delta = ffn; q.g.hi2_delta = 2 * ffn; }
        q.g.in_mul = pow2f(k_ln2); q.g.out_mul = pow2f(-k_h); q.g.range_amax = f16m ? slots + RS_H : nullptr;
        if (!gptj) block_ln(f, q, l.ln2_g, l.ln2_b, k_ln2, p_ln2, crest ? crest + RS_LN2 : nullptr);
        if ((st = launch16(f, EPI_BIAS_GELU, dt, q, "fc1")) != SGPT_OK) return st;
    }
    if (crest) launch_crest16(f.h, T, ffn, ldh, dt, crest + RS_H, s);
    if (m->calibrating) launch_absmax16(f.h, (long)T * ffn, dt, m->h_amax + li, s);
    QGemmArgs q{};
    q.g = proj(f, f.h, ldh, l.w_proj, dm, ffn, f.x, dm, l.b_proj, f.x);
    if (p_h) split_w(q.g, l.w_proj3, ffn);
    q.g.in_mul = pow2f(k_h);
    return launch16(f, EPI_BIAS_RESID, SGPT_F32, q, "fc2");
}

using BlockFn = sgpt_status (*)(const Fwd&, const LayerW&, int);
BlockFn pick_block(const Fwd& f) {
    const bool bf = f.dt != SGPT_F32;
    if (f.m->d.arch == SGPT_ARCH_BERT) return bf ? block_bert16 : block_bert_f32;
    if (f.m->d.arch == SGPT_ARCH_LLAMA) return bf ? block_llama16 : block_llama_f32;
    return f.mlp8 ? block_fp8 : (bf ? block_16 : block_f32);
}

sgpt_status check_call(sgpt_model* m, const int32_t* const (&layout)[4], const int32_t* pad_left, int B, int T, int max_alloc, int pool_mode,
                       int n_layers_run, bool pooled, const float* hidden_out) {
    sgpt_ctx* c = m->ctx;
    const Family& F = family(m->d.arch);
    if (!layout[0] || !layout[1] || !layout[2] || !layout[3] || B <= 0 || T <= 0 || T % 32 != 0 || max_alloc <= 0 || max_alloc % 2 != 0)
        return fail(c, SGPT_ERR_INVALID, "sgpt_encode: bad token layout (T_pad % 32, max_alloc_len % 2)");
    if (n_layers_run < 0 || n_layers_run > m->d.n_layers) return fail(c, SGPT_ERR_INVALID, "sgpt_encode: n_layers_run out of range");
    if (pool_mode < 0 || pool_mode > SGPT_POOL_CLS) return fail(c, SGPT_ERR_INVALID, "sgpt_encode: bad pool_mode");
    if (pool_mode == SGPT_POOL_LEARNTMEAN && !F.learntmean)
        return fail(c, SGPT_ERR_INVALID, std::string("sgpt_encode: learntmean pooling (trained position weights of the SGPT checkpoints) is not available for ") + F.name);
    if (pool_mode == SGPT_POOL_CLS && !F.cls) return fail(c, SGPT_ERR_INVALID, "sgpt_encode: cls pooling belongs to SGPT_ARCH_BERT");
    if (pool_mode == SGPT_POOL_LEARNTMEAN && pooled) {
        if (!m->pool_w) return fail(c, SGPT_ERR_MISSING, "sgpt_encode: learntmean needs sgpt_model_set_pool_weights first");
        if (!pad_left && max_alloc - 7 > m->pool_w_n)
            return fail(c, SGPT_ERR_INVALID, "sgpt_encode: fewer learnt position weights than the longest sequence");
    }
    if (max_alloc > 2048) return fail(c, SGPT_ERR_INVALID, "sgpt_encode: sequence longer than 2048 tokens");
    if (!pooled && !hidden_out) return fail(c, SGPT_ERR_INVALID, "sgpt_encode: no output requested");
    return SGPT_OK;
}

constexpr size_t SLACK = 64;

sgpt_status plan(Fwd& f, int n_layers_run, float** lp) {
    sgpt_model* m = f.m; sgpt_ctx* c = f.c;
    const int T = f.T, dm = m->d.d_model, ffn = m->d.d_ffn;
    const bool gptj = m->d.arch == SGPT_ARCH_GPTJ, fp8m = m->d.compute_dtype == SGPT_FP8M;
    const bool bf = m->d.compute_dtype != SGPT_F32;
    const size_t esz = bf ? 2 : 4;
    f.fp8 = m->d.compute_dtype == SGPT_FP8W || fp8m;
    f.dt = !bf ? SGPT_F32 : (m->d.compute_dtype == SGPT_F16 ? SGPT_F16 : SGPT_BF16);
    f.d_q = m->d.n_heads * head_dim(m->d); f.d_kv = m->d.n_kv_heads * head_dim(m->d);
    const size_t dq = f.d_q, dkv = f.d_kv;
    f.can_split = bf && !f.fp8;
    for (int li = 0; f.can_split && li < n_layers_run; ++li) {
        const int* pc = &m->prec[(size_t)li * PC_N];
        f.any_ln |= pc[PC_LN1] != 0 || pc[PC_LN2] != 0; f.any_att |= pc[PC_ATT] != 0; f.any_ctx |= pc[PC_CTX] != 0; f.any_h |= pc[PC_H] != 0;
    }
    f.split = f.any_ln || f.any_att || f.any_ctx || f.any_h;
    const bool shapes8 = gemm_fp8_shape_ok(T, ffn, dm) && gemm_fp8_shape_ok(T, dm, ffn) && gemm_fp8_shape_ok(T, 2 * dm, dm);
    f.mlp8 = fp8m && !m->calibrating && shapes8;
    if (f.mlp8)
        for (int li = 0; li < n_layers_run; ++li)
            if (!(m->act_scale[li] > 0.f) || !(m->act_scale[m->d.n_layers + li] > 0.f))
                return fail(c, SGPT_ERR_INVALID, "SGPT_FP8M: activation scales are not set (sgpt_model_calibrate_begin / _end, or sgpt_model_set_act_scales)");
    f.qpath = bf && !f.fp8 && !f.split && f.F->qpath && !(m->probing && m->crest_dev) && !m->calibrating && !c->force256 && !c->no_qpath && T <= QGEMM_MAX_ROWS &&
              qgemm_shape_ok(T, 3 * dm, dm, EPI_QKV, 2 * dm) && qgemm_shape_ok(T, dm, dm, EPI_BIAS_RESID, 0) &&
              qgemm_shape_ok(T, ffn, dm, EPI_BIAS_GELU, 0) && qgemm_shape_ok(T, dm, ffn, EPI_BIAS_RESID, 0);
    f.qln = f.qpath && !gptj && qgemm_ln_ok(T, 3 * dm, dm, EPI_QKV, 2 * dm) && qgemm_ln_ok(T, ffn, dm, EPI_BIAS_GELU, 0);
    size_t off = 0;
    auto carve = [&](size_t bytes) { size_t o = off; off = align_up(off + bytes, 256); return o; };
    const size_t o_x = carve((size_t)T * dm * 4);
    const size_t o_a = carve((size_t)T * (dq > (size_t)dm ? dq : (size_t)dm) * esz * (f.any_ln ? 3 : 1));
    const size_t o_c = (gptj || f.split) ? carve((size_t)T * dm * esz * (f.any_ctx ? 3 : 1)) : o_a;
    size_t qkv_elems = ((size_t)T + SLACK) * (dq + 2 * dkv);
    if (bf && ((size_t)T + 256) * (dq + dkv) > qkv_elems) qkv_elems = ((size_t)T + 256) * (dq + dkv);
    const size_t qkv_bytes = qkv_elems * esz;
    const size_t o_qkv = carve(qkv_bytes * (f.any_att ? 2 : 1));
    const size_t o_h = carve((size_t)T * ffn * esz * (f.any_h ? 3 : 1));
    const size_t o_gu = f.F->swiglu ? carve((size_t)T * 2 * ffn * esz) : 0;
    const size_t o_a8 = f.mlp8 ? carve((size_t)T * dm) : 0;
    const size_t o_sa = f.mlp8 ? carve((size_t)T * 4) : 0;
    const size_t o_lp = lp ? carve((size_t)(m->d.n_layers + 1) * f.B * dm * 4) : 0;
    sgpt_status st = ensure(c, &c->ws, &c->ws_bytes, off);
    if (st != SGPT_OK) return st;
    char* base = (char*)c->ws;
    f.range_flag = (f.mlp8 || f.dt == SGPT_F16) ? (int*)m->range_dev : nullptr;
    f.x = (float*)(base + o_x); f.a = base + o_a; f.ctx = base + o_c; f.qkv = base + o_qkv; f.h = base + o_h;
    if (f.F->swiglu) f.gu = base + o_gu;
    f.vt = bf ? (void*)((bf16_t*)f.qkv + ((size_t)T + SLACK) * (dq + dkv)) : nullptr;
    if (f.mlp8) { f.a8 = base + o_a8; f.sa = (float*)(base + o_sa); }
    if (lp) *lp = (float*)(base + o_lp);
    f.att_lo = (long)(qkv_bytes / 2);
    return SGPT_OK;
}

sgpt_status zero_overread(const Fwd& f) {
    sgpt_ctx* c = f.c; const size_t T = f.T, dm = f.m->d.d_model, dq = f.d_q, dkv = f.d_kv, esz = f.vt ? 2 : 4;
    if (f.vt)
        for (long lo = 0; lo <= (f.any_att ? f.att_lo : 0); lo += f.att_lo) {
            HIPC(c, hipMemsetAsync((bf16_t*)f.qkv + lo + T * (dq + dkv), 0, SLACK * (dq + dkv) * esz, f.s));
            HIPC(c, hipMemsetAsync((bf16_t*)f.vt + lo + T * dkv, 0, SLACK * dkv * esz, f.s));
        }
    else if (f.F->slack_f32) HIPC(c, hipMemsetAsync((float*)f.qkv + T * (dq + 2 * dkv), 0, SLACK * (dq + 2 * dkv) * esz, f.s));
    if (f.m->d.arch == SGPT_ARCH_GPTJ || f.mlp8 || f.split || f.qln || (f.F->post_ln && !f.vt))
        HIPC(c, hipMemsetAsync(f.ctx, 0, T * dm * esz * (f.any_ctx ? 3 : 1), f.s));
    else if (dq > dm) HIPC(c, hipMemsetAsync(f.ctx, 0, T * dq * esz, f.s));
    return SGPT_OK;
}

}

static sgpt_status encode_impl(sgpt_model* m, const int32_t* ids, const int32_t* pos, const int32_t* seq_off,
                               const int32_t* seq_len, const int32_t* pad_left, int32_t B, int32_t T, int32_t max_alloc,
                               int32_t pool_mode, int32_t n_layers_run, int32_t apply_final_ln, int32_t normalize,
                               float* out, float* hidden_out, float* layer_out, float* layer_mean, void* stream) {
    if (!m) return SGPT_ERR_INVALID;
    sgpt_ctx* c = m->ctx;
    const Family& F = family(m->d.arch);
    sgpt_status st = check_call(m, {ids, pos, seq_off, seq_len}, pad_left, B, T, max_alloc, pool_mode, n_layers_run, out || layer_out || layer_mean, hidden_out);
    if (st != SGPT_OK) return st;
    if (!F.lnf) apply_final_ln = 0;
    HIPC(c, hipSetDevice(c->device));
    hipStream_t s = (hipStream_t)stream;
    Fwd f{};
    f.m = m; f.c = c; f.s = s; f.F = &F; f.pos = pos; f.seq_off = seq_off; f.seq_len = seq_len; f.B = B; f.T = T; f.max_alloc = max_alloc;
    if ((st = plan(f, n_layers_run, layer_mean && !layer_out ? &layer_out : nullptr)) != SGPT_OK) return st;
    if ((st = zero_overread(f)) != SGPT_OK) return st;
    const int dm = m->d.d_model, ffn = m->d.d_ffn, dt = f.dt; float* x = f.x;
    auto pool = [&](int final_ln, float* dst, int* range_flag) {
        launch_lnf_pool(x, m->lnf_g, m->lnf_b, seq_off, seq_len, pad_left, B, dm, m->d.ln_eps, final_ln, pool_mode, normalize, m->pool_w,
                        m->pool_w_n, dst, s, range_flag, F.norm_kind);
    };
    launch_embed(ids, pos, m->wte, m->wpe, x, T, dm, m->d.vocab, m->d.max_pos, s);
    if (F.post_ln && f.vt) launch_layernorm_writeback(x, m->emb_ln_g, m->emb_ln_b, f.a, dt, T, dm, m->d.ln_eps, f.range_flag, s);
    else if (m->emb_ln_g) launch_layernorm(x, m->emb_ln_g, m->emb_ln_b, x, SGPT_F32, T, dm, m->d.ln_eps, s);
    const BlockFn block = pick_block(f);
    for (int li = 0; li < n_layers_run; ++li) {
        LayerW l = m->L[li];
        if (layer_out) pool(0, layer_out + (size_t)li * B * dm, nullptr);
        if (f.fp8 && !f.mlp8) {
            launch_fp8_dequant_rows(l.w_qkv, l.s_qkv, (long)3 * dm, dm, m->dq[0], SGPT_BF16, s);
            launch_fp8_dequant_rows(l.w_o, l.s_o, dm, dm, m->dq[1], SGPT_BF16, s);
            launch_fp8_dequant_rows(l.w_fc, l.s_fc, ffn, dm, m->dq[2], SGPT_BF16, s);
            launch_fp8_dequant_rows(l.w_proj, l.s_proj, dm, ffn, m->dq[3], SGPT_BF16, s);
            l.w_qkv = m->dq[0]; l.w_o = m->dq[1]; l.w_fc = m->dq[2]; l.w_proj = m->dq[3];
        }
        if ((st = block(f, l, li)) != SGPT_OK) return st;
    }
    if (hidden_out) {
        if (apply_final_ln && F.norm_kind == 1) launch_rmsnorm(x, m->lnf_g, hidden_out, SGPT_F32, T, dm, m->d.ln_eps, nullptr, s);
        else if (apply_final_ln) launch_layernorm(x, m->lnf_g, m->lnf_b, hidden_out, SGPT_F32, T, dm, m->d.ln_eps, s);
        else HIPC(c, hipMemcpyAsync(hidden_out, x, (size_t)T * dm * 4, hipMemcpyDeviceToDevice, s));
    }
    if (out) pool(apply_final_ln, out, m->d.compute_dtype == SGPT_F16 ? (int*)m->range_dev : nullptr);
    if (layer_out) pool(apply_final_ln, layer_out + (size_t)n_layers_run * B * dm, nullptr);
    if (layer_mean) launch_mean_over_axis0(layer_out, n_layers_run + 1, (long)B * dm, layer_mean, s);
    HIPC(c, hipGetLastError());
    return SGPT_OK;
}

extern "C" {

sgpt_status sgpt_encode(sgpt_model* m, const int32_t* ids, const int32_t* pos, const int32_t* seq_off,
                        const int32_t* seq_len, const int32_t* pad_left, int32_t B, int32_t T, int32_t max_alloc,
                        int32_t pool_mode, int32_t n_layers_run, int32_t apply_final_ln, int32_t normalize,
                        float* out, float* hidden_out, void* stream) {
    return encode_impl(m, ids, pos, seq_off, seq_len, pad_left, B, T, max_alloc, pool_mode, n_layers_run,
                       apply_final_ln, normalize, out, hidden_out, nullptr, nullptr, stream);
}

sgpt_status sgpt_encode_layers(sgpt_model* m, const int32_t* ids, const int32_t* pos, const int32_t* seq_off,
                               const int32_t* seq_len, const int32_t* pad_left, int32_t B, int32_t T, int32_t max_alloc,
                               int32_t pool_mode, int32_t normalize, float* out_layers, float* out_mean, void* stream) {
    if (!m) return SGPT_ERR_INVALID;
    if (!out_layers && !out_mean) return fail(m->ctx, SGPT_ERR_INVALID, "sgpt_encode_layers: no output requested");
    return encode_impl(m, ids, pos, seq_off, seq_len, pad_left, B, T, max_alloc, pool_mode, m->d.n_layers, 1, normalize,
                       nullptr, nullptr, out_layers, out_mean, stream);
}

sgpt_status sgpt_lm_logprobs(sgpt_model* m, const float* hidden, const int32_t* row_idx, const int32_t* targets,
                             int32_t n, float* out_logprob, int32_t* out_greedy, void* stream) {
    if (!m) return SGPT_ERR_INVALID;
    sgpt_ctx* c = m->ctx;
    if (!hidden || !row_idx || !targets || !out_logprob || n <= 0) return fail(c, SGPT_ERR_INVALID, "sgpt_lm_logprobs: bad arguments");
    if (family(m->d.arch).no_lm) return fail(c, SGPT_ERR_INVALID, std::string("sgpt_lm_logprobs: ") + family(m->d.arch).no_lm);
    HIPC(c, hipSetDevice(c->device));
    hipStream_t s = (hipStream_t)stream;
    const int dm = m->d.d_model, V = m->d.vocab;
    const long ldv = (V + 3) / 4 * 4;
    const int R = n < 1024 ? n : 1024;
    const size_t rows_bytes = align_up((size_t)R * dm * 4, 256), lg_bytes = align_up((size_t)R * ldv * 4, 256);
    sgpt_status st = ensure(c, &c->ws2, &c->ws2_bytes, rows_bytes + lg_bytes);
    if (st != SGPT_OK) return st;
    float* rows = (float*)c->ws2;
    float* logits = (float*)((char*)c->ws2 + rows_bytes);
    for (int r0 = 0; r0 < n; r0 += R) {
        const int nr = (n - r0) < R ? (n - r0) : R;
        launch_gather_rows(hidden, row_idx + r0, nr, dm, rows, s);
        GemmArgs g{};
        g.A = rows; g.lda = dm; g.W = m->lm_w; g.ldw = dm; g.M = nr; g.m_valid = nr; g.N = V; g.K = dm;
        g.out = logits; g.ldo = ldv; g.bias = m->lm_b;
        gemm(c, SGPT_F32, EPI_STORE, SGPT_F32, g, s);
        launch_logprob_rows(logits, ldv, V, targets + r0, nr, out_logprob + r0, out_greedy ? out_greedy + r0 : nullptr, s);
    }
    HIPC(c, hipGetLastError());
    return SGPT_OK;
}

}
```

### sgpt_amd/csrc/gemm.hip

```cpp
#include <cstdlib>

#include "common.h"
#include "score64_epilogue.h"
#include "score_plan.h"

namespace {

#ifndef SGPT_RESID_NT
#define SGPT_RESID_NT 0
#endif
constexpr bool RESID_NT = SGPT_RESID_NT != 0;
#ifndef SGPT_RESID_LD_NT
#define SGPT_RESID_LD_NT 0
#endif
constexpr bool RESID_LD_NT = SGPT_RESID_LD_NT != 0;
#ifndef SGPT_FOLD_TAIL_SCORE
#define SGPT_FOLD_TAIL_SCORE 1
#endif
#ifndef SGPT_FOLD_TAIL
#define SGPT_FOLD_TAIL 1
#endif
#ifndef SGPT_THV_UNCOND
#define SGPT_THV_UNCOND 1
#endif
// ... 726 lines not shown
                    const int row = wave * 32 + j * 16 + fr;
                    df[j] = ld[row * CH + ((4 * ks + g) ^ (row & 7))];
                }
#pragma unroll
                for (int i = 0; i < 4; ++i) {
                    const int row = i * 16 + fr;
                    qf[i] = lq[row * CH + ((4 * ks + g) ^ (row & 7))];
                }
#pragma unroll
                for (int i = 0; i < 4; ++i)
#pragma unroll
                    for (int j = 0; j < 2; ++j) mma<T, true>(acc[i][j], qf[i], df[j]);
            }
            ss ^= 1;
            sd = sd + 1 >= 3 ? 0 : sd + 1;
        }
        float thv[4] = {INFINITY, INFINITY, INFINITY, INFINITY};
        if constexpr (EPI == EPI_SCORE_FILTER) {
#pragma unroll
            for (int i = 0; i < 4; ++i)
                if (i * 16 + fr < p.m_valid) thv[i] = p.thr[(long)(i * 16 + fr) * p.thr_ld];
        }
        score64_epilogue<EPI, false>(p, acc, thv, (long)tile * 256 + wave * 32, g, fr, lane,
                                     reinterpret_cast<uint2_a*>(stage_all) + (EPI == EPI_SCORE_FILTER ? wave * 256 : 0));
        if (!has_next) break;
        tile = ntile; dsrc = ndsrc;
    }
    asm volatile("s_waitcnt vmcnt(0)" ::: "memory");
}

template <typename T, int EPI>
void launch_score64(const GemmArgs& a, hipStream_t s) {
    const int ncu = device_cu_count();
    const int NT = a.N / 256;
    hipLaunchKernelGGL((score64_kernel<T, EPI>), dim3(NT < ncu ? NT : ncu), dim3(512), 0, s, a);
}

template <typename T, int EPI, typename OutT, bool SWAP>
void launch(const GemmArgs& a, hipStream_t s) {
    const long t128 = (long)((a.M + 127) / 128) * ((a.N + 127) / 128);
    static const long t128_env = exp_env("SGPT_T128_MIN") ? atol(exp_env("SGPT_T128_MIN")) : -1;
    const long t128_min = t128_env >= 0 ? t128_env : (a.K <= 1024 ? 600 : 300);
    const bool small = t128 < t128_min;
    const int B = small ? 64 : 128;
    const int MT = (a.M + B - 1) / B, NT = (a.N + B - 1) / B;
    const int mt_per_xcd = (MT + 7) / 8;
    const int bands = (mt_per_xcd + 7) / 8;
    const int grid = (long)MT * NT <= 512 ? 8 * ((MT * NT + 7) / 8) : 8 * bands * 8 * NT;
    const long tiles = (long)MT * NT;
    const bool deep = small && tiles <= SGPT_DEEP_TILES;
    const int kgmax = a.kgroups;
    constexpr bool splittable = EPI != EPI_SCORE && EPI != EPI_SCORE_FILTER;
    constexpr int EPC = ElemTraits<T>::EPC;
    const int nkt16 = (a.K + 16 * EPC - 1) / (16 * EPC);
    if constexpr (splittable) {
        if (deep && kgmax >= 2) {
            if (nkt16 % 2 == 0 && nkt16 / 2 >= SGPT_KG16_MIN) {
                hipLaunchKernelGGL((gemm_kernel<T, EPI, OutT, SWAP, 2, 2, 16>), dim3(grid), dim3(512), 0, s, a); return;
            }
        }
    }
    if (deep) hipLaunchKernelGGL((gemm_kernel<T, EPI, OutT, SWAP, 2, 1, 16>), dim3(grid), dim3(256), 0, s, a);
    else if (small) hipLaunchKernelGGL((gemm_kernel<T, EPI, OutT, SWAP, 2, 1, 8>), dim3(grid), dim3(256), 0, s, a);
    else hipLaunchKernelGGL((gemm_kernel<T, EPI, OutT, SWAP, 4, 1, 8>), dim3(grid), dim3(256), 0, s, a);
}

template <typename H>
void launch_gemm16(int epi, int out_dtype, const GemmArgs& a, hipStream_t s) {
    const bool o16 = dt_is16(out_dtype);
    if (a.n_valid > 0) {
        const bool scorer_ = epi == EPI_SCORE || epi == EPI_SCORE_FILTER || epi == EPI_SCORE_TOP2;
        if (!(scorer_ && gemm_score_tail_foldable(a.M, a.N, a.K))) {
            const int whole = a.N - 256;
            GemmArgs b = a;
            b.N = whole; b.n_valid = 0;
            if (whole > 0) launch_gemm16<H>(epi, out_dtype, b, s);
            GemmArgs t = a;
            t.W = static_cast<const char*>(a.W) + (size_t)whole * a.ldw * 2; t.N = a.n_valid - whole; t.n_valid = 0;
            if (a.out != nullptr) t.out = static_cast<float*>(a.out) + whole;
            t.idx_base = a.idx_base + whole;
            if (t.N > 0) launch_gemm16<H>(epi, out_dtype, t, s);
            return;
        }
    }
    static const bool small_tiles = exp_env("SGPT_NO_SMALL_TILE") == nullptr;
    const bool scorer = epi == EPI_SCORE || epi == EPI_SCORE_FILTER || epi == EPI_SCORE_TOP2;
    const long few_limit = epi_is_gelu(epi) ? 255 : SGPT_FEW_TILES;
    const bool few = small_tiles && !a.force256 && !scorer && (long)(a.M / 256) * (a.N / 256) <= few_limit;
    static const bool use256 = exp_env("SGPT_GEMM128") == nullptr;
    const bool shape256 = a.M % 256 == 0 && a.N % 256 == 0 && a.K % 64 == 0 && a.K >= 128;
    if (scorer && a.M == 64 && a.N % 256 == 0 && a.K % 64 == 0 && a.K >= 128) {
        if (epi == EPI_SCORE) return launch_score64<H, EPI_SCORE>(a, s);
        return launch_score64<H, EPI_SCORE_FILTER>(a, s);
    }
    if (epi == EPI_SCORE_FILTER && !shape256) return launch<H, EPI_SCORE_FILTER, float, true>(a, s);
    if (epi == EPI_QKV) {
        if (gemm_qkv_bulk(a.M, a.N, a.K, a.n_split, a.force256 != 0) && a.lda == a.ldw && a.bias == nullptr && a.lo_delta == 0 &&
            a.lo_delta2 == 0 && a.m_valid == a.M) {
            GemmArgs b = a;
#if defined(SGPT_QKV_GM) && defined(SGPT_QKV_GN)
            b.gm = SGPT_QKV_GM; b.gn = SGPT_QKV_GN;
#endif
            return launch256d<H, EPI_QKV, H, true>(b, s, true);
        }
        return launch<H, EPI_QKV, H, true>(a, s);
    }
    if (use256 && shape256 && (scorer || (!few && a.m_valid == a.M))) {
        const bool deep_a = a.M >= a.N;
#ifdef SGPT_EXPERIMENTS
        if (g_use_w && (epi != EPI_STORE || o16))
            return launch_gemm256w(Half<H>::is_f16 ? DT_F16 : DT_BF16, epi, a, s, deep_a);
#endif
        if (a.lo_delta != 0) {
            if (epi == EPI_STORE && o16) return launch256d<H, EPI_STORE, H, true, true>(a, s, deep_a);
            if (epi == EPI_VT) return launch256d<H, EPI_VT, H, false, true>(a, s, deep_a);
            if (epi == EPI_BIAS_GELU) return launch256d<H, EPI_BIAS_GELU, H, true, true>(a, s, deep_a);
            abort();
        }
        if (epi == EPI_SCORE) return launch256d<H, EPI_SCORE, float, true>(a, s, deep_a);
        if (epi == EPI_SCORE_FILTER) return launch256d<H, EPI_SCORE_FILTER, float, true>(a, s, deep_a);
        if (epi == EPI_SCORE_TOP2) return launch256d<H, EPI_SCORE_TOP2, float, true>(a, s, deep_a);
        if (epi == EPI_STORE && o16) return launch256d<H, EPI_STORE, H, true>(a, s, deep_a);
        if (epi == EPI_VT) return launch256d<H, EPI_VT, H, false>(a, s, deep_a);
        if (epi == EPI_BIAS_GELU) return launch256d<H, EPI_BIAS_GELU, H, true>(a, s, deep_a);
        if (epi == EPI_BIAS_GELU_ERF) return launch256d<H, EPI_BIAS_GELU_ERF, H, true>(a, s, deep_a);
        if (epi == EPI_BIAS_RESID) return launch256d<H, EPI_BIAS_RESID, float, true>(a, s, deep_a);
        if (epi == EPI_NONE) return launch256d<H, EPI_NONE, H, true>(a, s, deep_a);
    }
    if (epi == EPI_STORE && o16) return launch<H, EPI_STORE, H, true>(a, s);
    if (epi == EPI_STORE && !o16) return launch<H, EPI_STORE, float, true>(a, s);
    if (epi == EPI_VT) return launch<H, EPI_VT, H, false>(a, s);
    if (epi == EPI_BIAS_GELU) return launch<H, EPI_BIAS_GELU, H, true>(a, s);
    if (epi == EPI_BIAS_GELU_ERF) return launch<H, EPI_BIAS_GELU_ERF, H, true>(a, s);
    if (epi == EPI_BIAS_RESID) return launch<H, EPI_BIAS_RESID, float, true>(a, s);
    if (epi == EPI_SCORE) return launch<H, EPI_SCORE, float, true>(a, s);
    abort();
}

}

bool gemm_qkv_one_launch(int M, int n_split, bool force256) {
    static const bool small_tiles = exp_env("SGPT_NO_SMALL_TILE") == nullptr && exp_env("SGPT_QKV_TWO") == nullptr;
    return small_tiles && !force256 && n_split % 128 == 0 && (long)(M / 256) * (n_split / 256) * 2 <= 256;
}
#ifndef SGPT_QKV_BULK
#define SGPT_QKV_BULK 1
#endif
bool gemm_qkv_bulk(int M, int N, int K, int n_split, bool force256) {
    (void)force256;
    if (!SGPT_QKV_BULK || exp_env("SGPT_QKV_TWO") != nullptr || exp_env("SGPT_GEMM128") != nullptr) return false;
    return M % 256 == 0 && N % 256 == 0 && n_split % 256 == 0 && n_split < N && K % 64 == 0 && K >= 128 &&
           (long)(M / 256) * (n_split / 256) > SGPT_FEW_TILES;
}
bool gemm_score_tail_foldable(int M, long N, int K) {
    if (exp_env("SGPT_GEMM128") != nullptr) return false;
    return score_tail_foldable_shape(M, N, K);
}
#ifdef SGPT_EXPERIMENTS
int set_gemm_skew(int cycles) { const int old = g_skew; g_skew = cycles; return old; }
int set_gemm_use_w(int on) { const int old = g_use_w; g_use_w = on ? 1 : 0; return old; }
#endif

void launch_gemm(int dtype, int epi, int out_dtype, const GemmArgs& a0, hipStream_t s) {
    GemmArgs a = a0;
    if (a.in_mul == 0.f) a.in_mul = 1.f;
    if (a.out_mul == 0.f) a.out_mul = 1.f;
    if (a.out_mul2 == 0.f) a.out_mul2 = 1.f;
    if (a.kgroups < 1) a.kgroups = 1;
    if (dtype == DT_BF16) return launch_gemm16<bf16_t>(epi, out_dtype, a, s);
    if (dtype == DT_F16) return launch_gemm16<f16_t>(epi, out_dtype, a, s);
    if (epi == EPI_STORE) return launch<float, EPI_STORE, float, true>(a, s);
    if (epi == EPI_BIAS_GELU) return launch<float, EPI_BIAS_GELU, float, true>(a, s);
    if (epi == EPI_BIAS_GELU_ERF) return launch<float, EPI_BIAS_GELU_ERF, float, true>(a, s);
    if (epi == EPI_BIAS_RESID) return launch<float, EPI_BIAS_RESID, float, true>(a, s);
    if (epi == EPI_SCORE) return launch<float, EPI_SCORE, float, true>(a, s);
    abort();
}
```

### sgpt_amd/model.py

```python
import ctypes as C
import itertools
import json
import os
from dataclasses import dataclass
from typing import Dict, List, Optional, Sequence, Tuple

import numpy as np
import torch

from . import _lib
from ._lib import (ModelDesc, TensorView, POOL_MODES, SGPT_BF16, SGPT_F16, SGPT_F32, SGPT_FP8M, SGPT_FP8W, SgptRangeError,
                   SGPT_PREC_CLASSES, PC_LN1, PC_ATT, PC_CTX, PC_LN2, PC_H)
from .families import (MAX_SEQ_LEN, SGPTConfig, alibi_slopes, bert_state_dict, family, head_dim, llama_state_dict, rotary_tables,
                       rotary_tables_half, synthetic_bert_weights, synthetic_llama_weights, synthetic_qwen_weights, synthetic_weights)
from .runtime import Context, get_context, _p, _stream_ptr

CREST_LIMIT_LN = 12.0
CREST_LIMIT_H = 20.0
PROBE_MAX_ROWS = 8192

ALIGN = 2
TOKEN_TILE = 256
QUERY_ROWS = 512
QUERY_TILE = 32


def pad_rows(total: int, row_tile: Optional[int] = None) -> int:
    tile = row_tile or (QUERY_TILE if total <= QUERY_ROWS else TOKEN_TILE)
    return (int(total) + tile - 1) // tile * tile


@dataclass
class PackedBatch:
    ids: torch.Tensor
    pos: torch.Tensor
    seq_off: torch.Tensor
    seq_len: torch.Tensor
    pad_left: torch.Tensor
    B: int
    T_pad: int
    max_alloc: int
    n_tokens: int
    max_pos: int = 0
    arena: Optional[torch.Tensor] = None
    n_real: int = 0


def _flatten(seqs, total: int) -> np.ndarray:
    if isinstance(seqs, np.ndarray) and seqs.ndim == 2:
        return _to_i32(seqs).reshape(-1)
    if len(seqs) and isinstance(seqs[0], np.ndarray):
        return _to_i32(np.concatenate(seqs))
    return np.fromiter(itertools.chain.from_iterable(seqs), dtype=np.int32, count=total)


def _to_i32(a: np.ndarray) -> np.ndarray:
    if a.dtype != np.int32 and a.size and (int(a.max()) > np.iinfo(np.int32).max or int(a.min()) < np.iinfo(np.int32).min):
        raise ValueError("token id out of range")
    return np.ascontiguousarray(a, dtype=np.int32)


def pack_layout(seqs, pad_left: Optional[Sequence[int]] = None, bucket: Optional[Tuple[int, int, int]] = None,
                row_tile: Optional[int] = None) -> dict:
    B = len(seqs)
    if isinstance(seqs, np.ndarray) and seqs.ndim == 2:
        lens = np.full(B, seqs.shape[1], dtype=np.int64)
    else:
        lens = np.fromiter(map(len, seqs), dtype=np.int64, count=B)
    if B == 0 or (lens <= 0).any():
        raise ValueError("Empty items should be cleaned prior to running")
    pl = np.zeros(B, dtype=np.int32) if pad_left is None else np.asarray(pad_left, dtype=np.int32)
    n_real, n_tokens = B, int(lens.sum())
    max_pos = int((lens + pl.astype(np.int64)).max()) - 1
    if bucket is not None:
        B_cap, T_cap, A_cap = bucket
        if B_cap < B or T_cap != pad_rows(T_cap, row_tile) or A_cap % ALIGN:
            raise ValueError(f"bucket {bucket} cannot hold {B} sequences (T_cap % {TOKEN_TILE}, or % {QUERY_TILE} up to "
                             f"{QUERY_ROWS} rows; A_cap % {ALIGN})")
        lens = np.concatenate([lens, np.ones(B_cap - B, dtype=np.int64)])
        pl = np.concatenate([pl, np.zeros(B_cap - B, dtype=np.int32)])
        B = B_cap
    alloc = (lens + ALIGN - 1) // ALIGN * ALIGN
    off = np.zeros(B + 1, dtype=np.int64)
    np.cumsum(alloc, out=off[1:])
    T_pad = pad_rows(int(off[-1]), row_tile)
    max_alloc = int(alloc.max())
    if bucket is not None:
        if T_pad > bucket[1] or max_alloc > bucket[2]:
            raise ValueError(f"packed layout (T_pad {T_pad}, max_alloc {max_alloc}) does not fit bucket {bucket}")
        T_pad, max_alloc = bucket[1], bucket[2]
    return dict(B=B, lens=lens, alloc=alloc, off=off, T_pad=T_pad, pl=pl, n_tokens=n_tokens, n_real=n_real,
                max_alloc=max_alloc, max_pos=max_pos)


def arena_ints(lay: dict) -> int:
    return 2 * lay["T_pad"] + 3 * lay["B"] + 1


def fill_arena(seqs, lay: dict, arena: np.ndarray):
    B, T_pad, lens, off, pl = lay["B"], lay["T_pad"], lay["lens"], lay["off"], lay["pl"]
    n = lay["n_tokens"]
    ids, pos = arena[:T_pad], arena[T_pad: 2 * T_pad]
    ids[:] = 0
    pos[:] = 0
    flat = _flatten(seqs, n)
    if flat.shape[0] != n:
        raise ValueError("ragged token input does not match its lengths")
    hi_lo = (int(flat.max()), int(flat.min()))
    if B > lay["n_real"]:
        flat = np.concatenate([flat, np.zeros(B - lay["n_real"], dtype=np.int32)])
        n = flat.shape[0]
    if (lens == lens[0]).all() and lens[0] % ALIGN == 0:
        ids[:n] = flat
        pos[:n] = (np.arange(n, dtype=np.int64) % lens[0] + np.repeat(pl.astype(np.int64), lens)).astype(np.int32)
    else:
        within = np.arange(n, dtype=np.int64) - np.repeat(np.cumsum(lens) - lens, lens)
        rows = np.repeat(off[:-1], lens) + within
        ids[rows] = flat
        pos[rows] = (within + np.repeat(pl.astype(np.int64), lens)).astype(np.int32)
    o = 2 * T_pad
    arena[o: o + B + 1] = off
    arena[o + B + 1: o + 2 * B + 1] = lens
    arena[o + 2 * B + 1: o + 3 * B + 1] = pl
    return hi_lo


def pack_host(seqs: Sequence[Sequence[int]], pad_left: Optional[Sequence[int]] = None,
              bucket: Optional[Tuple[int, int, int]] = None):
    lay = pack_layout(seqs, pad_left, bucket)
    arena = np.empty(arena_ints(lay), dtype=np.int32)
    fill_arena(seqs, lay, arena)
    B, T_pad = lay["B"], lay["T_pad"]
    o = 2 * T_pad
    return dict(ids=arena[:T_pad], pos=arena[T_pad:o], seq_off=arena[o: o + B + 1], seq_len=arena[o + B + 1: o + 2 * B + 1],
                pad_left=arena[o + 2 * B + 1: o + 3 * B + 1], B=B, T_pad=T_pad, max_alloc=lay["max_alloc"],
                n_tokens=lay["n_tokens"], max_pos=lay["max_pos"], n_real=lay["n_real"], arena=arena)


class _Staging:

    def __init__(self, device):
        self.device = device
        self.bufs = [None, None]
        self.events = [None, None]
        self.turn = 0

    def acquire(self, n_int: int):
        i = self.turn
        self.turn ^= 1
        if self.events[i] is not None:
            self.events[i].synchronize()
        if self.bufs[i] is None or self.bufs[i].numel() < n_int:
            cap = max(n_int + n_int // 4, 1 << 16)
            self.bufs[i] = torch.empty(cap, dtype=torch.int32).pin_memory()
        return i, self.bufs[i]

    def release(self, i: int):
        ev = self.events[i] or torch.cuda.Event()
        ev.record(torch.cuda.current_stream(self.device))
        self.events[i] = ev


PRECISE_QK_PLANS = {"full": (1, 0, 0), "logits": (0, 1, 0), "act+logits": (3, 1, 0), "full+logits": (1, 1, 0),
                    "qkv+logits": (2, 1, 0), "attn": (2, 1, 1)}


def default_precise_qk(cfg: "SGPTConfig", dtype: str):
    if dtype != "f16" or family(cfg.model_type).scaled_logits or cfg.hidden_size < 2048:
        return False
    if head_dim(cfg) not in (64, 128):
        return "full"
    return "act+logits" if cfg.hidden_size < 2560 else "qkv+logits"


def check_args(cfg: SGPTConfig, dtype: str, precise_qk, precision):
    fam = family(cfg.model_type)
    if dtype in ("fp16", "float16", "half"):
        dtype = "f16"
    if precision is None:
        precision = "auto" if (dtype == "f16" and fam.sgpt_modes) else "plain"
    if precision not in ("plain", "x3", "auto", "auto-class"):
        raise ValueError("precision must be 'plain', 'x3', 'auto' or 'auto-class'")
    if precision != "plain" and dtype not in ("f16", "bf16"):
        raise ValueError("precision applies to dtype 'f16' / 'bf16'")
    if precise_qk is None:
        precise_qk = default_precise_qk(cfg, dtype)
    if precise_qk is True:
        precise_qk = "full"
    if precise_qk not in (False,) + tuple(PRECISE_QK_PLANS):
        raise ValueError(f"precise_qk must be None, False, True or one of {sorted(PRECISE_QK_PLANS)}")
    if precise_qk and dtype not in ("f16", "bf16"):
        raise ValueError("precise_qk applies to dtype 'f16' / 'bf16'")
    if not fam.sgpt_modes and dtype in ("fp8", "fp8mfma"):
        raise ValueError(f"dtype {dtype!r} is not available for {fam.name} models: use {fam.dtype_advice}")
    if not fam.sgpt_modes and (precision != "plain" or precise_qk):
        raise ValueError(f"split-precision operands (precision='x3' / 'auto' / 'auto-class', precise_qk) are not available for {fam.name} models")
    if fam.grouped_kv and cfg.num_heads % cfg.num_kv_heads:
        raise ValueError("num_heads must be a multiple of num_kv_heads")
# ... 108 lines not shown
        alloc = np.cumsum((lens + ALIGN - 1) // ALIGN * ALIGN)
        n = max(1, int(np.searchsorted(alloc, PROBE_MAX_ROWS, side="right")))
        sub = [seqs[i][:PROBE_MAX_ROWS] for i in range(n)]
        pl = None if pad_left is None else [pad_left[i] for i in range(n)]
        out = (C.c_float * (4 * self.cfg.num_layers))()

        def once():
            self._call("precision_probe_begin")
            try:
                self.encode_packed(self.pack(sub, pl))
            finally:
                self._call("precision_probe_end", out)
        self.guarded(once)
        return np.array(list(out), dtype=np.float32).reshape(self.cfg.num_layers, 4)

    def ensure_precision_plan(self, seqs, pad_left=None) -> None:
        if self._plan_pending:
            self._auto_precision(seqs, pad_left)

    def release_split_weights(self) -> int:
        plan = self.precision_plan()
        if plan[:, [PC_CTX, PC_LN2, PC_H]].any():
            return 0
        freed = C.c_int64(0)
        self._call("release_split_weights", C.byref(freed))
        return int(freed.value)

    def sync_precision(self, seqs, reduce, pad_left=None) -> None:
        if self.precision not in ("auto", "auto-class") or self.dtype not in ("f16", "bf16"):
            return
        L = self.cfg.num_layers
        flags = np.zeros(L * 4 + 3, dtype=np.int32)
        crest = None
        if self._plan_pending:
            crest = self.probe_precision(seqs, pad_left)
            flags[: L * 4] = (crest > self._crest_limits()[None, :]).reshape(-1)
            flags[L * 4] = 1
        rep = self.precision_report or {}
        flags[L * 4 + 1] = 1 if rep.get("decided", "plain") != "plain" else 0
        flags[L * 4 + 2] = 1 if (not self._plan_pending and rep.get("split_weight_bytes_released", 0) > 0) else 0
        tot = np.asarray(reduce(flags.copy()), dtype=np.int32)
        if tot[L * 4] == 0 and tot[L * 4 + 1] == flags[L * 4 + 1]:
            return
        hot = tot[: L * 4].reshape(L, 4) > 0
        if tot[L * 4 + 1] and not hot.any():
            hot[:] = True
        if hot.any() and tot[L * 4 + 2]:
            raise RuntimeError(
                f"sync_precision: the collective probe asks for split-precision operands ({int(hot.sum())} (block, class) flags over "
                f"the ranks), but {int(tot[L * 4 + 2])} rank(s) already settled on plain operands in an earlier call and released "
                "their split weight copies.  Raised on every rank.  Load the models with precision='x3' (or pin one plan with "
                "set_precision_plan() on every rank) before a multi-process search over this data.")
        self._install_from_flags(hot, crest, probed="first call (collective)")

    def _crest_limits(self) -> np.ndarray:
        return np.array([CREST_LIMIT_LN, CREST_LIMIT_LN, CREST_LIMIT_LN, CREST_LIMIT_H], dtype=np.float32)

    def _install_from_flags(self, hot: np.ndarray, crest, probed: str, final: bool = True) -> None:
        plan = self._base_plan()
        if hot.any():
            if self.precision == "auto":
                plan = self._x3_plan()
            else:
                plan[hot[:, 0], PC_LN1] = 2
                if self._att_ok:
                    plan[hot[:, 0], PC_ATT] = 1
                plan[hot[:, 1], PC_CTX] = 1
                plan[hot[:, 2], PC_LN2] = 1
                plan[hot[:, 3], PC_H] = 1
                if family(self.cfg.model_type).parallel_block:
                    plan[:, PC_LN2] = (plan[:, PC_LN1] != 0).astype(np.int32)
            self.set_precision_plan(plan)
        freed = 0
        if final:
            self._plan_pending = False
            if not hot.any():
                freed = self.release_split_weights()
        self.precision_report = dict(crest=crest, limits=self._crest_limits().tolist(), flagged=int(hot.sum()), probed=probed,
                                     decided="x3" if (hot.any() and self.precision == "auto") else ("classes" if hot.any() else "plain"),
                                     split_weight_bytes_released=freed)

    def _auto_precision(self, seqs, pad_left, final: bool = True) -> None:
        if final:
            self._plan_pending = False
        crest = self.probe_precision(seqs, pad_left)
        hot = crest > self._crest_limits()[None, :]
        self._install_from_flags(hot, crest, probed="first call" if final else "load (synthetic)", final=final or bool(hot.any()))

    def calibrate(self, seqs: Optional[Sequence[Sequence[int]]] = None, margin: float = 2.0) -> np.ndarray:
        if self.dtype != "fp8mfma":
            raise ValueError("calibrate() applies to dtype='fp8mfma'")
        if seqs is None:
            import warnings
            warnings.warn("dtype='fp8mfma': activation scales calibrated on 64 synthetic random-token sequences; pass representative "
                          "token lists to SGPTModel.calibrate() (a later batch that saturates the e4m3 range raises SgptRangeError)",
                          stacklevel=2)
            S = min(64, self.cfg.max_position_embeddings)
            seqs = np.random.default_rng(1234).integers(0, self.cfg.vocab_size, size=(64, S), dtype=np.int64)
        self._call("calibrate_begin")
        try:
            self.encode_ids(seqs)
        finally:
            out = (C.c_float * (2 * self.cfg.num_layers))()
            self._call("calibrate_end", float(margin), out)
        self.act_scales = np.array(list(out), dtype=np.float32)
        return self.act_scales

    def set_act_scales(self, scales) -> None:
        a = np.ascontiguousarray(scales, dtype=np.float32)
        self._call("set_act_scales", a.ctypes.data_as(C.c_void_p), a.size)
        self.act_scales = a

    def set_position_weights(self, w) -> None:
        t = w if isinstance(w, torch.Tensor) else torch.from_numpy(np.ascontiguousarray(w))
        t = t.detach().to(device=self.device, dtype=torch.float32).contiguous().reshape(-1)
        self._call("set_pool_weights", _p(t), t.numel())
        self.position_weights = t

    def close(self):
        if getattr(self, "handle", None):
            self.ctx.lib.sgpt_model_free(self.handle)
            self.handle = None

    @classmethod
    def from_pretrained(cls, path: str, **kw) -> "SGPTModel":
        root = path
        if not os.path.exists(os.path.join(root, "config.json")) and os.path.exists(os.path.join(root, "0_Transformer")):
            root = os.path.join(root, "0_Transformer")
        with open(os.path.join(root, "config.json")) as f:
            cfg = SGPTConfig.from_hf_dict(json.load(f))
        model = cls(cfg, load_state_dict(root), **kw)
        wmp = os.path.join(path, "1_WeightedMeanPooling", "pytorch_model.bin")
        if os.path.exists(wmp):
            model.set_position_weights(torch.load(wmp, map_location="cpu", weights_only=True)["position_weights"])
        return model

    def pack(self, seqs: Sequence[Sequence[int]], pad_left: Optional[Sequence[int]] = None,
             bucket: Optional[Tuple[int, int, int]] = None, into: Optional[PackedBatch] = None) -> PackedBatch:
        lay = pack_layout(seqs, pad_left, bucket, self.row_tile)
        if lay["max_alloc"] > 2048 or lay["max_pos"] >= self.cfg.max_position_embeddings:
            raise ValueError("sequence longer than max_position_embeddings")
        n_int = arena_ints(lay)
        B, T = lay["B"], lay["T_pad"]
        if into is not None and (into.arena is None or (into.B, into.T_pad, into.max_alloc) != (B, T, lay["max_alloc"])):
            raise ValueError(f"packed layout {(B, T, lay['max_alloc'])} does not match the batch being refilled "
                             f"{(into.B, into.T_pad, into.max_alloc)}")
        slot, host = self._staging.acquire(n_int)
        hi, lo = fill_arena(seqs, lay, host.numpy())
        if lo < 0 or hi >= self.cfg.vocab_size:
            raise ValueError(f"token id out of range [0, {self.cfg.vocab_size})")
        dev = into.arena if into is not None else torch.empty(n_int, dtype=torch.int32, device=self.device)
        dev.copy_(host[:n_int], non_blocking=True)
        self._staging.release(slot)
        if into is not None:
            into.n_tokens, into.max_pos, into.n_real = lay["n_tokens"], lay["max_pos"], lay["n_real"]
            return into
        o = 2 * T
        return PackedBatch(dev[:T], dev[T:o], dev[o: o + B + 1], dev[o + B + 1: o + 2 * B + 1],
                           dev[o + 2 * B + 1: o + 3 * B + 1], B, T, lay["max_alloc"], lay["n_tokens"], lay["max_pos"],
                           arena=dev, n_real=lay["n_real"])

    def encode_packed(self, pb: PackedBatch, mode: str = "weightedmean", normalize: bool = False,
                      layer_idx: int = -1, out: Optional[torch.Tensor] = None,
                      return_hidden: bool = False):
        if mode not in POOL_MODES:
            raise ValueError(f"unknown pooling mode {mode}")
        L = self.cfg.num_layers
        li = layer_idx if layer_idx >= 0 else L + 1 + layer_idx
        if not 0 <= li <= L:
            raise ValueError(f"Layer Idx {layer_idx} is larger than the {L + 1} hidden states")
        n_run, final_ln = (L, 1) if li == L else (li, 0)
        self._check_learnt(mode, pb)
        d = self.cfg.hidden_size
        if out is None:
            out = torch.empty((pb.B, d), dtype=torch.float32, device=self.device)
        hidden = torch.empty((pb.T_pad, d), dtype=torch.float32, device=self.device) if return_hidden else None
        st = self.ctx.lib.sgpt_encode(self.handle, _p(pb.ids), _p(pb.pos), _p(pb.seq_off), _p(pb.seq_len),
                                      _p(pb.pad_left), pb.B, pb.T_pad, pb.max_alloc, POOL_MODES[mode], n_run,
                                      final_ln, 1 if normalize else 0, _p(out), _p(hidden),
                                      _stream_ptr(self.device))
        _lib.check(self.ctx.handle, st, "sgpt_encode")
        return (out, hidden) if return_hidden else out

    def _check_learnt(self, mode: str, pb: PackedBatch) -> None:
        if mode != "learntmean":
            return
        if not family(self.cfg.model_type).sgpt_modes:
            raise ValueError("method 'learntmean' (trained position weights of the SGPT checkpoints) is not available for BERT / Llama models")
        if self.position_weights is None:
            raise ValueError("method 'learntmean' needs trained position weights (1_WeightedMeanPooling)")
        if pb.max_pos >= self.position_weights.numel():
            raise ValueError("fewer learnt position weights than the longest padded sequence")

    def encode_packed_layers(self, pb: PackedBatch, mode: str = "mean", normalize: bool = False,
                             per_layer: bool = False):
        if mode not in POOL_MODES:
            raise ValueError(f"unknown pooling mode {mode}")
        self._check_learnt(mode, pb)
        d, L1 = self.cfg.hidden_size, self.cfg.num_layers + 1
        layers = torch.empty((L1, pb.B, d), dtype=torch.float32, device=self.device) if per_layer else None
        mean = torch.empty((pb.B, d), dtype=torch.float32, device=self.device)
        st = self.ctx.lib.sgpt_encode_layers(self.handle, _p(pb.ids), _p(pb.pos), _p(pb.seq_off), _p(pb.seq_len),
                                             _p(pb.pad_left), pb.B, pb.T_pad, pb.max_alloc, POOL_MODES[mode],
                                             1 if normalize else 0, _p(layers), _p(mean), _stream_ptr(self.device))
        _lib.check(self.ctx.handle, st, "sgpt_encode_layers")
        return (layers, mean) if per_layer else mean

    def lm_logprobs(self, hidden: torch.Tensor, row_idx, targets, return_greedy: bool = False):
        if refusal := family(self.cfg.model_type).no_lm_head:
            raise ValueError(refusal)
        ri = torch.as_tensor(np.asarray(row_idx, dtype=np.int32)).to(self.device)
        tg = torch.as_tensor(np.asarray(targets, dtype=np.int32)).to(self.device)
        n = int(ri.numel())
        out = torch.empty((n,), dtype=torch.float32, device=self.device)
        greedy = torch.empty((n,), dtype=torch.int32, device=self.device) if return_greedy else None
        hidden = hidden.contiguous()
        st = self.ctx.lib.sgpt_lm_logprobs(self.handle, _p(hidden), _p(ri), _p(tg), n, _p(out), _p(greedy),
                                           _stream_ptr(self.device))
        _lib.check(self.ctx.handle, st, "sgpt_lm_logprobs")
        return (out, greedy) if return_greedy else out

    def _num_cus(self) -> int:
        try:
            return int(torch.cuda.get_device_properties(self.device).multi_processor_count) // 8 * 8 or 256
        except Exception:
            return 256

    def call_budgets(self, total_rows: int, ncu: Optional[int] = None) -> List[int]:
        ncu = ncu or self._num_cus()
        d, ffn = self.cfg.hidden_size, self.cfg.intermediate_size
        nt_d = max(1, d // TOKEN_TILE)
        mt_max = max(1, self.max_tokens_per_call // TOKEN_TILE)
        mt_tot = -(-int(total_rows) // TOKEN_TILE)
        if mt_tot <= mt_max:
            return [mt_tot * TOKEN_TILE]
        launches = [(3 * d // TOKEN_TILE, d), (nt_d, d), (max(1, ffn // TOKEN_TILE), d), (nt_d, ffn)]
        per_row = 0.35 * sum(nt * k for nt, k in launches) / ncu

        def cost(mt):
            return sum(-(-mt * nt // ncu) * k for nt, k in launches) + per_row * mt

        good = sorted({min(mt_max, j * ncu // nt_d) for j in range(1, mt_max * nt_d // ncu + 2)} | {mt_max})
        good = [g for g in good if g >= 1]
        n_min = -(-mt_tot // mt_max)
        best, cands = None, []
        for n_calls in (n_min, n_min + 1):
            n_free = min(n_calls, 3 if n_calls == n_min else 4)
            fixed = n_calls - n_free
            rem = mt_tot - fixed * mt_max
            if rem <= 0:
                continue
            for combo in itertools.combinations_with_replacement(good, n_free - 1):
                last = rem - sum(combo)
                if last <= 0 or last > mt_max:
                    continue
                c = fixed * cost(mt_max) + sum(cost(g) for g in combo) + cost(last)
                cands.append((c, [mt_max] * fixed + sorted(combo, reverse=True) + [last]))
        if cands:
            c_min = min(c for c, _ in cands)
            best = max((pl for c, pl in cands if c <= c_min * 1.003), key=lambda pl: (min(pl), -len(pl)))
        if best is None:
            best = [mt_max] * (n_min - 1) + [mt_tot - (n_min - 1) * mt_max]
        return [b * TOKEN_TILE for b in best]

    def plan_batches(self, lens: np.ndarray, max_sentences: Optional[int] = None) -> List[np.ndarray]:
        order = np.argsort(-lens, kind="stable")
        alloc = (lens[order] + ALIGN - 1) // ALIGN * ALIGN
        total = int(alloc.sum())
        round_aware = getattr(self, "round_aware_calls", True)
        if not round_aware:
            n_calls = max(1, -(-total // self.max_tokens_per_call))
            equal = min(self.max_tokens_per_call, (-(-total // n_calls) + TOKEN_TILE - 1) // TOKEN_TILE * TOKEN_TILE + int(alloc.max()))

        def budget_for(remaining: int) -> int:
            if not round_aware:
                return equal
            b = self.call_budgets(remaining)
            return self.max_tokens_per_call if len(b) == 1 else min(self.max_tokens_per_call, b[0])
        out, start, tok, done = [], 0, 0, 0
        budget = budget_for(total)
        for i, a in enumerate(alloc):
            full = tok + a > budget or (max_sentences and i - start >= max_sentences)
            if full and i > start:
                out.append(order[start:i])
                done += tok
                start, tok = i, 0
                budget = budget_for(total - done)
            tok += int(a)
        out.append(order[start:])
        return out

    def range_flags(self, reset: bool = True) -> int:
        flagged = C.c_int32(0)
        self._call("range_check", C.byref(flagged), 1 if reset else 0, _stream_ptr(self.device))
        return int(flagged.value)

    def range_shifts(self) -> np.ndarray:
        out = np.zeros(self.cfg.num_layers * 4, dtype=np.int32)
        self._call("get_range_shifts", out.ctypes.data_as(C.c_void_p), out.size)
        return out.reshape(self.cfg.num_layers, 4)

    def set_range_shifts(self, shifts) -> None:
        a = np.ascontiguousarray(np.asarray(shifts, dtype=np.int32).reshape(-1))
        self._call("set_range_shifts", a.ctypes.data_as(C.c_void_p), a.size)

    def _adapt_range(self) -> bool:
        n = C.c_int32(0)
        self._call("range_adapt", C.byref(n), _stream_ptr(self.device))
        return n.value > 0

    def check_range(self, adapt: bool = False) -> bool:
        if self.dtype not in ("f16", "fp8mfma"):
            return False
        flags = self.range_flags(reset=False)
        if not flags:
            return False
        if flags & 1 and not flags & 6 and adapt and self.dtype == "f16" and family(self.cfg.model_type).sgpt_modes and self._adapt_range():
            return True
        self.range_flags(reset=True)
        if flags & 2:
            raise SgptRangeError("dtype='fp8mfma': a GELU output saturated its e4m3 codes; re-run calibrate() on "
                                 "representative inputs (or with a larger margin)")
        if flags & 4:
            raise SgptRangeError("dtype='fp8mfma': an attention context saturated its e4m3 codes; re-run calibrate() on "
                                 "representative inputs (or with a larger margin)")
        raise SgptRangeError("dtype='f16': an activation reached |v| >= 32768 (IEEE-half range)" +
                             (" and no range shift covers it; this checkpoint needs dtype='bf16'" if adapt else
                              "; re-run the call under SGPTModel.guarded / check_range(adapt=True)"))

    _check_range = check_range

    def guarded(self, fn):
        for _ in range(8):
# ... 127 lines not shown
```

### sgpt_amd/runtime.py

```python
import ctypes as C
from typing import Optional, Tuple

import numpy as np
import torch

from . import _lib
from ._lib import SGPT_BF16, SGPT_F16, SGPT_F32, POOL_MODES
from .corpus import CORPUS_KINDS, RESCORE_MODES, BinaryCorpus, CorpusBuilders, QuantizedCorpus, Uint8Corpus, _no_rescore

DT_CODE = {torch.float32: SGPT_F32, torch.bfloat16: SGPT_BF16, torch.float16: SGPT_F16}


def _stream_ptr(device) -> C.c_void_p:
    return C.c_void_p(torch.cuda.current_stream(device).cuda_stream)


def _p(t: Optional[torch.Tensor]) -> C.c_void_p:
    return C.c_void_p(0 if t is None else t.data_ptr())


_contexts = {}


def get_context(device=None) -> "Context":
    if not torch.cuda.is_available():
        raise _lib.SgptHipError("no HIP device visible: sgpt_amd runs its hot path only as gfx950 kernels "
                                "(there is no CPU path)")
    dev = torch.device("cuda", torch.cuda.current_device()) if device is None else torch.device(device)
    if dev.type != "cuda":
        raise _lib.SgptHipError(f"sgpt_amd needs a HIP device, got {dev}")
    idx = dev.index if dev.index is not None else torch.cuda.current_device()
    if idx not in _contexts:
        _contexts[idx] = Context(idx)
    return _contexts[idx]


class Context(CorpusBuilders):

    def __init__(self, device_index: int):
        self.lib = _lib.load()
        self.device = torch.device("cuda", device_index)
        h = C.c_void_p()
        st = self.lib.sgpt_ctx_create(device_index, C.byref(h))
        if st != 0:
            raise _lib.SgptHipError(f"sgpt_ctx_create(device={device_index}) failed with status {st}")
        self.handle = h

    def close(self):
        if getattr(self, "handle", None):
            self.lib.sgpt_ctx_destroy(self.handle)
            self.handle = None

    def _chk(self, st, what):
        _lib.check(self.handle, st, what)

    def _dev_f32(self, a) -> torch.Tensor:
        if not isinstance(a, torch.Tensor):
            a = torch.as_tensor(np.asarray(a))
        if a.dim() == 1:
            a = a.unsqueeze(0)
        return a.to(device=self.device, dtype=torch.float32).contiguous()

    def _run_list(self, run, nq: int, k: int) -> Tuple[torch.Tensor, torch.Tensor, int]:
        if run is not None:
            return run
        return (torch.empty((nq, k), dtype=torch.float32, device=self.device),
                torch.empty((nq, k), dtype=torch.int64, device=self.device), 0)

    def _u8_operands(self, corpus: Uint8Corpus) -> Tuple[torch.Tensor, torch.Tensor, torch.Tensor]:
        return (corpus.codes.to(self.device).contiguous(), corpus.start.to(device=self.device, dtype=torch.float32).contiguous(),
                corpus.step.to(device=self.device, dtype=torch.float32).contiguous())

    def pool(self, hidden: torch.Tensor, mask: torch.Tensor, mode: str = "weightedmean",
             position_weights: Optional[torch.Tensor] = None) -> torch.Tensor:
        if mode not in POOL_MODES:
            raise ValueError(f"unknown pooling mode {mode}")
        hidden = hidden.to(self.device)
        if hidden.dtype not in DT_CODE:
            hidden = hidden.float()
        hidden = hidden.contiguous()
        B, S, d = hidden.shape
        m = mask.to(device=self.device, dtype=torch.int32).contiguous()
        out = torch.empty((B, d), dtype=torch.float32, device=self.device)
        dt = DT_CODE[hidden.dtype]
        if mode == "learntmean":
            if position_weights is None or position_weights.numel() < S:
                raise ValueError("learntmean needs position_weights covering the sequence length")
            pw = position_weights.to(device=self.device, dtype=torch.float32).contiguous()
            self._chk(self.lib.sgpt_pool_learnt(self.handle, _p(hidden), dt, _p(m), B, S, d, _p(pw), _p(out),
                                                _stream_ptr(self.device)), "sgpt_pool_learnt")
            return out
        self._chk(self.lib.sgpt_pool(self.handle, _p(hidden), dt, _p(m), B, S, d, POOL_MODES[mode], _p(out),
                                     _stream_ptr(self.device)), "sgpt_pool")
        return out

    def l2_normalize(self, x: torch.Tensor, out_dtype=torch.float32) -> torch.Tensor:
        x = self._dev_f32(x)
        n, d = x.shape
        out = torch.empty((n, d), dtype=out_dtype, device=self.device)
        self._chk(self.lib.sgpt_l2_normalize(self.handle, _p(x), n, d, _p(out), DT_CODE[out_dtype],
                                             _stream_ptr(self.device)), "sgpt_l2_normalize")
        return out

    def pairwise_scores(self, a: torch.Tensor, b: torch.Tensor, cosine: bool) -> torch.Tensor:
        a, b = self._dev_f32(a), self._dev_f32(b)
        if a.shape != b.shape or a.dim() != 2:
            raise ValueError(f"pairwise scores need two [n, d] matrices of one shape, got {tuple(a.shape)} and {tuple(b.shape)}")
        n, d = a.shape
        out = torch.empty((n,), dtype=torch.float32, device=self.device)
        if n:
            self._chk(self.lib.sgpt_pairwise_scores(self.handle, _p(a), _p(b), n, d, 1 if cosine else 0, _p(out),
                                                    _stream_ptr(self.device)), "sgpt_pairwise_scores")
        return out

    def to_16(self, x: torch.Tensor, dtype=torch.float16, out: Optional[torch.Tensor] = None) -> torch.Tensor:
        x = x.to(device=self.device, dtype=torch.float32).contiguous()
        if out is None:
            out = torch.empty(x.shape, dtype=dtype, device=self.device)
        self._chk(self.lib.sgpt_f32_to_16(self.handle, _p(x), x.numel(), _p(out), DT_CODE[dtype],
                                          _stream_ptr(self.device)), "sgpt_f32_to_16")
        return out

    def row_crest(self, x: torch.Tensor) -> float:
        if x.dtype not in (torch.float16, torch.bfloat16):
            x = self.to_16(self._dev_f32(x), torch.float16)
        x = x.to(self.device).contiguous()
        n, d = x.shape
        out = C.c_float(0)
        self._chk(self.lib.sgpt_row_crest(self.handle, _p(x), DT_CODE[x.dtype], n, d, d, C.byref(out),
                                          _stream_ptr(self.device)), "sgpt_row_crest")
        return float(out.value)

    def split16(self, x: torch.Tensor, role: str, dtype=torch.float16) -> torch.Tensor:
        if role not in ("doc", "query"):
            raise ValueError("role must be 'doc' or 'query'")
        x = self._dev_f32(x)
        n, d = x.shape
        out = torch.empty((n, 3 * d), dtype=dtype, device=self.device)
        self._chk(self.lib.sgpt_split16(self.handle, _p(x), n, d, 0 if role == "doc" else 1, _p(out), DT_CODE[dtype],
                                        _stream_ptr(self.device)), "sgpt_split16")
        return out

    def to_bf16(self, x: torch.Tensor) -> torch.Tensor:
        return self.to_16(x, torch.bfloat16)

    def range_check(self, reset: bool = True) -> int:
        flagged = C.c_int32(0)
        self._chk(self.lib.sgpt_range_check(self.handle, C.byref(flagged), 1 if reset else 0, _stream_ptr(self.device)),
                  "sgpt_range_check")
        return int(flagged.value)

    def generation(self) -> int:
        return int(self.lib.sgpt_ctx_generation(self.handle))

    def set_low_latency(self, on: bool) -> bool:
        return bool(self.lib.sgpt_ctx_set_low_latency(self.handle, 1 if on else 0))

    def set_gemm_cu_cap(self, n: int) -> int:
        return int(self.lib.sgpt_ctx_set_gemm_cu_cap(self.handle, int(n)))

    def set_tile_policy(self, force_256) -> int:
        return int(self.lib.sgpt_ctx_set_tile_policy(self.handle, int(force_256)))

    def set_query_tile(self, k: int) -> int:
        return int(self.lib.sgpt_ctx_set_query_tile(self.handle, int(k)))

    def reserve(self, encode_bytes: int = 0, score_bytes: int = 0) -> None:
        self._chk(self.lib.sgpt_ctx_reserve(self.handle, encode_bytes, score_bytes), "sgpt_ctx_reserve")

    def fp8_quantize_rows(self, w: torch.Tensor) -> Tuple[torch.Tensor, torch.Tensor]:
        w = w.to(device=self.device, dtype=torch.float32).contiguous()
        rows, cols = w.shape
        codes = torch.empty((rows, cols), dtype=torch.uint8, device=self.device)
        scale = torch.empty((rows,), dtype=torch.float32, device=self.device)
        self._chk(self.lib.sgpt_fp8_quantize_rows(self.handle, _p(w), rows, cols, _p(codes), _p(scale),
                                                  _stream_ptr(self.device)), "sgpt_fp8_quantize_rows")
        return codes, scale

    def fp8_dequantize_rows(self, codes: torch.Tensor, scale: torch.Tensor, out_dtype=torch.float32) -> torch.Tensor:
        codes = codes.to(device=self.device, dtype=torch.uint8).contiguous()
        scale = scale.to(device=self.device, dtype=torch.float32).contiguous()
        rows, cols = codes.shape
        out = torch.empty((rows, cols), dtype=out_dtype, device=self.device)
        self._chk(self.lib.sgpt_fp8_dequantize_rows(self.handle, _p(codes), _p(scale), rows, cols, _p(out),
                                                    DT_CODE[out_dtype],
                                                    _stream_ptr(self.device)), "sgpt_fp8_dequantize_rows")
        return out

    def score_overflow_count(self) -> Tuple[int, int]:
        a, b = C.c_int32(0), C.c_int32(0)
        self._chk(self.lib.sgpt_score_overflow_count(self.handle, C.byref(a), C.byref(b), _stream_ptr(self.device)),
                  "sgpt_score_overflow_count")
        return int(a.value), int(b.value)

    def _operand(self, x: torch.Tensor, dtype) -> torch.Tensor:
        if x.dtype == dtype and x.device == self.device and x.is_contiguous():
            return x
        if dtype in (torch.bfloat16, torch.float16):
            return self.to_16(x, dtype)
        return x.to(device=self.device, dtype=torch.float32).contiguous()

    def linear(self, a: torch.Tensor, w: torch.Tensor, bias: Optional[torch.Tensor] = None, epi: str = "store",
               resid: Optional[torch.Tensor] = None, out_dtype=None) -> torch.Tensor:
        code = {"store": 0, "gelu": 1, "resid": 2, "vt": 4, "gelu_erf": 9}[epi]
        M, K = a.shape
        N = w.shape[0]
        if out_dtype is None:
            out_dtype = torch.float32 if epi == "resid" else a.dtype
        out = torch.empty((N, M) if epi == "vt" else (M, N), dtype=out_dtype, device=self.device)
        b = None if bias is None else bias.to(device=self.device, dtype=torch.float32).contiguous()
        r = None if resid is None else resid.to(device=self.device, dtype=torch.float32).contiguous()
        self._chk(self.lib.sgpt_linear(self.handle, DT_CODE[a.dtype], code, DT_CODE[out_dtype], _p(a.contiguous()),
                                       _p(w.contiguous()), _p(b), _p(r), _p(out), M, N, K, _stream_ptr(self.device)),
                  "sgpt_linear")
        return out

    def linear_query(self, w: torch.Tensor, a: Optional[torch.Tensor] = None, x: Optional[torch.Tensor] = None, ln=None,
                     bias: Optional[torch.Tensor] = None, epi: str = "store", resid: Optional[torch.Tensor] = None, n_split: int = 0):
        code = {"store": 0, "gelu": 1, "resid": 2, "qkv": 7}[epi]
        N, K = w.shape
        src = a if a is not None else x
        M = src.shape[0]
        odt = torch.float32 if epi == "resid" else w.dtype
        out = torch.empty((M, n_split if epi == "qkv" else N), dtype=odt, device=self.device)
        vt = torch.empty((N - n_split, M), dtype=odt, device=self.device) if epi == "qkv" else None
        f32 = lambda t_: None if t_ is None else t_.to(device=self.device, dtype=torch.float32).contiguous()
        g, b, eps = (f32(ln[0]), f32(ln[1]), float(ln[2])) if ln is not None else (None, None, 0.0)
        b32, r32, x32 = f32(bias), f32(resid), f32(x)
        self._chk(self.lib.sgpt_linear_query(self.handle, DT_CODE[w.dtype], code, _p(None if a is None else a.contiguous()), _p(x32), _p(g), _p(b), eps,
                                             _p(w.contiguous()), _p(b32), _p(r32), _p(out), _p(vt), int(n_split), M, N, K,
                                             _stream_ptr(self.device)), "sgpt_linear_query")
        return (out, vt) if epi == "qkv" else out

    def linear_qkv(self, a: torch.Tensor, w: torch.Tensor, n_split: int):
        M, K = a.shape
        N = w.shape[0]
        out = torch.empty((M, n_split), dtype=a.dtype, device=self.device)
        vt = torch.empty((N - n_split, M), dtype=a.dtype, device=self.device)
        self._chk(self.lib.sgpt_linear_qkv(self.handle, DT_CODE[a.dtype], _p(a.contiguous()), _p(w.contiguous()), _p(out), _p(vt),
                                           int(n_split), M, N, K, _stream_ptr(self.device)), "sgpt_linear_qkv")
        return out, vt

    def linear_split(self, a: torch.Tensor, w: torch.Tensor, bias: Optional[torch.Tensor] = None, epi: str = "store",
                     triple: bool = False) -> torch.Tensor:
        code = {"store": 0, "gelu": 1, "vt": 4}[epi]
        M, K = a.shape
        N = w.shape[0]
        b = None if bias is None else bias.to(device=self.device, dtype=torch.float32).contiguous()
        if epi == "vt":
            out = torch.zeros((2, N, M), dtype=a.dtype, device=self.device)
            ldo, lo, hi2 = M, N * M, 0
        else:
            out = torch.zeros((M, (3 if triple else 2) * N), dtype=a.dtype, device=self.device)
            ldo, lo, hi2 = out.shape[1], N, (2 * N if triple else 0)
        self._chk(self.lib.sgpt_linear_split(self.handle, DT_CODE[a.dtype], code, _p(a.contiguous()), _p(w.contiguous()), _p(b),
                                             _p(out), ldo, lo, hi2, M, N, K, _stream_ptr(self.device)), "sgpt_linear_split")
        return out

    def attention(self, q: torch.Tensor, k: torch.Tensor, v: torch.Tensor, out: torch.Tensor, seq_off: torch.Tensor,
                  H: int, dh: int, max_alloc_len: int, window: int = 0, scale: float = 1.0, alibi: Optional[torch.Tensor] = None,
                  out_scale: float = 0.0, range_flag: Optional[torch.Tensor] = None, x3: bool = False, qk_lo_delta: int = 0,
                  v_lo_delta: int = 0, ctx_lo_delta: int = 0, ctx_hi2_delta: int = 0, causal: Optional[bool] = None,
                  seq_len: Optional[torch.Tensor] = None, n_kv_heads: Optional[int] = None) -> torch.Tensor:
        T = q.shape[0]
        out_fp8 = out.dtype == torch.uint8
        if q.dtype not in DT_CODE:
            raise ValueError(f"attention: operands are fp32, bf16 or f16, got {q.dtype}")
        if k.stride(0) != q.stride(0) or q.stride(1) != 1 or k.stride(1) != 1 or v.stride(1) != 1 or out.stride(1) != 1:
            raise ValueError("attention: q and k share one leading dimension; unit column strides")
        if k.dtype != q.dtype or v.dtype != q.dtype:
            raise ValueError("attention: q, k and v have one dtype")
        if out.dtype != q.dtype and not (out_fp8 and q.dtype == torch.bfloat16):
            raise ValueError("attention: out has q's dtype (or uint8 e4m3 codes for bf16 operands)")
        if q.dtype == torch.float32 and v.stride(0) != q.stride(0):
            raise ValueError("attention: fp32 v rows share q's leading dimension (the fp32 kernel reads v with ldq)")
        so = seq_off.to(device=self.device, dtype=torch.int32).contiguous()
        al = None if alibi is None else alibi.to(device=self.device, dtype=torch.float32).contiguous()
        if n_kv_heads is not None:
            if causal is False or seq_len is not None:
                raise ValueError("attention: grouped K / V is causal")
            self._chk(self.lib.sgpt_attention_gqa(self.handle, DT_CODE[q.dtype], _p(q), _p(k), _p(v), q.stride(0), v.stride(0), _p(out),
                                                  out.stride(0), _p(so), so.numel() - 1, T, H, int(n_kv_heads), dh, window, scale, _p(al),
                                                  max_alloc_len, 1 if out_fp8 else 0, out_scale, _p(range_flag), 1 if x3 else 0,
                                                  qk_lo_delta, v_lo_delta, ctx_lo_delta, ctx_hi2_delta, _stream_ptr(self.device)),
                      "sgpt_attention_gqa")
            return out
        if causal is not None:
            sl = None if seq_len is None else seq_len.to(device=self.device, dtype=torch.int32).contiguous()
            self._chk(self.lib.sgpt_attention_ex(self.handle, DT_CODE[q.dtype], _p(q), _p(k), _p(v), q.stride(0), v.stride(0), _p(out),
                                                 out.stride(0), _p(so), so.numel() - 1, T, H, dh, window, scale, _p(al), max_alloc_len,
                                                 1 if out_fp8 else 0, out_scale, _p(range_flag), 1 if x3 else 0, qk_lo_delta,
                                                 v_lo_delta, ctx_lo_delta, ctx_hi2_delta, 1 if causal else 0, _p(sl),
                                                 _stream_ptr(self.device)), "sgpt_attention_ex")
            return out
        self._chk(self.lib.sgpt_attention(self.handle, DT_CODE[q.dtype], _p(q), _p(k), _p(v), q.stride(0), v.stride(0), _p(out),
                                          out.stride(0), _p(so), so.numel() - 1, T, H, dh, window, scale, _p(al), max_alloc_len,
                                          1 if out_fp8 else 0, out_scale, _p(range_flag), 1 if x3 else 0, qk_lo_delta,
                                          v_lo_delta, ctx_lo_delta, ctx_hi2_delta, _stream_ptr(self.device)), "sgpt_attention")
        return out

    def _f32c(self, t: Optional[torch.Tensor]) -> Optional[torch.Tensor]:
        return None if t is None else t.to(device=self.device, dtype=torch.float32).contiguous()

    def embed(self, ids: torch.Tensor, pos: Optional[torch.Tensor], wte: torch.Tensor, wpe: Optional[torch.Tensor] = None,
              vocab: Optional[int] = None, max_pos: Optional[int] = None, out: Optional[torch.Tensor] = None) -> torch.Tensor:
        T, d = ids.numel(), wte.shape[1]
        if wte.stride() != (d, 1) or (wpe is not None and wpe.stride() != (d, 1)):
            raise ValueError("embed: tables are row-contiguous [rows, d]")
        if out is None:
            out = torch.empty((T, d), dtype=torch.float32, device=self.device)
        self._chk(self.lib.sgpt_embed(self.handle, _p(ids), _p(pos), _p(wte), _p(wpe), T, d,
                                      wte.shape[0] if vocab is None else int(vocab),
                                      (wpe.shape[0] if wpe is not None else 0) if max_pos is None else int(max_pos), _p(out),
                                      _stream_ptr(self.device)), "sgpt_embed")
        return out

    def layernorm(self, x: torch.Tensor, gamma: torch.Tensor, beta: torch.Tensor, eps: float = 1e-5, out_dtype=torch.float32,
                  out_mul: float = 1.0, split: bool = False, out: Optional[torch.Tensor] = None) -> torch.Tensor:
# ... 339 lines not shown
```

Before: 37950.

## Split large encode batches into two phase-offset stream chains for overlap

Large packed encode batches are cut at a 256-aligned sequence boundary near the middle. The two halves run through all layers on separate HIP streams, with the second chain's start delayed by half a layer so their kernels interleave. This aims to fill idle compute units left by serialized per-layer kernels and tail effects. It adds a second stream, events, a memset to clear overread regions at the cut, and a host copy of sequence offsets. It only applies to big, 256-divisible, non-captured, pooled-only runs.

```diff
diff --git a/include/sgpt_hip.h b/include/sgpt_hip.h
--- a/include/sgpt_hip.h
+++ b/include/sgpt_hip.h
@@ -8,7 +8,7 @@
 extern "C" {
 #endif
 
-#define SGPT_ABI_VERSION 21
+#define SGPT_ABI_VERSION 22
 
 typedef int sgpt_status;
 #define SGPT_OK 0
@@ -71,6 +71,12 @@
                         int32_t B, int32_t T_pad, int32_t max_alloc_len,
                         int32_t pool_mode, int32_t n_layers_run, int32_t apply_final_ln,
                         int32_t normalize, float* out, float* hidden_out, void* stream);
+
+sgpt_status sgpt_encode_host_layout(sgpt_model* model, const int32_t* ids, const int32_t* pos,
+                                    const int32_t* seq_off, const int32_t* seq_len, const int32_t* pad_left,
+                                    int32_t B, int32_t T_pad, int32_t max_alloc_len,
+                                    int32_t pool_mode, int32_t n_layers_run, int32_t apply_final_ln,
+                                    int32_t normalize, float* out, float* hidden_out, const int32_t* seq_off_host, void* stream);
 
 sgpt_status sgpt_encode_layers(sgpt_model* model, const int32_t* ids, const int32_t* pos,
                                const int32_t* seq_off, const int32_t* seq_len, const int32_t* pad_left,
@@ -280,6 +286,8 @@
 sgpt_status sgpt_prof_enable(sgpt_ctx* ctx, int32_t on);
 sgpt_status sgpt_prof_read(sgpt_ctx* ctx, int64_t* launches, double* ms, double* flops, int32_t reset);
 
+int32_t sgpt_ctx_set_encode_chains(sgpt_ctx* ctx, int32_t n, int32_t min_rows);
+int64_t sgpt_ctx_encode_chain_calls(const sgpt_ctx* ctx);
 int32_t sgpt_ctx_set_gemm_cu_cap(sgpt_ctx* ctx, int32_t n);
 int32_t sgpt_ctx_set_low_latency(sgpt_ctx* ctx, int32_t on);
 int32_t sgpt_ctx_set_tile_policy(sgpt_ctx* ctx, int32_t policy);
diff --git a/sgpt_amd/_lib.py b/sgpt_amd/_lib.py
--- a/sgpt_amd/_lib.py
+++ b/sgpt_amd/_lib.py
@@ -5,7 +5,7 @@
 LIB_PATH = os.environ.get("SGPT_HIP_LIB") or os.path.join(HERE, "lib", "libsgpt_hip.so")
 
 SGPT_F32, SGPT_BF16, SGPT_FP8W, SGPT_F16, SGPT_FP8M = 0, 1, 2, 3, 4
-SGPT_ABI_VERSION = 21
+SGPT_ABI_VERSION = 22
 SGPT_PREC_CLASSES = 5
 PC_LN1, PC_ATT, PC_CTX, PC_LN2, PC_H = 0, 1, 2, 3, 4
 SGPT_ERR_RANGE = -5
@@ -43,6 +43,9 @@
     "sgpt_encode": (C.c_int, [C.c_void_p, C.c_void_p, C.c_void_p, C.c_void_p, C.c_void_p, C.c_void_p,
                               C.c_int32, C.c_int32, C.c_int32, C.c_int32, C.c_int32, C.c_int32, C.c_int32,
                               C.c_void_p, C.c_void_p, C.c_void_p]),
+    "sgpt_encode_host_layout": (C.c_int, [C.c_void_p, C.c_void_p, C.c_void_p, C.c_void_p, C.c_void_p, C.c_void_p,
+                                          C.c_int32, C.c_int32, C.c_int32, C.c_int32, C.c_int32, C.c_int32, C.c_int32,
+                                          C.c_void_p, C.c_void_p, C.c_void_p, C.c_void_p]),
     "sgpt_encode_layers": (C.c_int, [C.c_void_p, C.c_void_p, C.c_void_p, C.c_void_p, C.c_void_p, C.c_void_p,
                                      C.c_int32, C.c_int32, C.c_int32, C.c_int32, C.c_int32, C.c_void_p, C.c_void_p,
                                      C.c_void_p]),
@@ -135,6 +138,8 @@
     "sgpt_ctx_set_tile_policy": (C.c_int32, [C.c_void_p, C.c_int32]),
     "sgpt_ctx_set_gemm_cu_cap": (C.c_int32, [C.c_void_p, C.c_int32]),
     "sgpt_ctx_set_query_tile": (C.c_int32, [C.c_void_p, C.c_int32]),
+    "sgpt_ctx_set_encode_chains": (C.c_int32, [C.c_void_p, C.c_int32, C.c_int32]),
+    "sgpt_ctx_encode_chain_calls": (C.c_int64, [C.c_void_p]),
     "sgpt_model_range_check": (C.c_int, [C.c_void_p, C.POINTER(C.c_int32), C.c_int32, C.c_void_p]),
     "sgpt_model_range_adapt": (C.c_int, [C.c_void_p, C.POINTER(C.c_int32), C.c_void_p]),
     "sgpt_model_get_range_shifts": (C.c_int, [C.c_void_p, C.c_void_p, C.c_int32]),
diff --git a/sgpt_amd/csrc/common.h b/sgpt_amd/csrc/common.h
--- a/sgpt_amd/csrc/common.h
+++ b/sgpt_amd/csrc/common.h
@@ -274,6 +274,7 @@
 bool gemm_qkv_one_launch(int M, int n_split, bool force256);
 bool gemm_score_tail_foldable(int M, long N, int K);
 bool gemm_qkv_bulk(int M, int N, int K, int n_split, bool force256);
+bool gemm_bulk_256(int M, int N, int K, int epi, bool force256);
 #ifdef SGPT_EXPERIMENTS
 int set_gemm_skew(int cycles);
 int set_gemm_use_w(int on);
diff --git a/sgpt_amd/csrc/ctx.h b/sgpt_amd/csrc/ctx.h
--- a/sgpt_amd/csrc/ctx.h
+++ b/sgpt_amd/csrc/ctx.h
@@ -24,6 +24,10 @@
     int no_qpath = 0;
     int cu_cap = 0;
     int qtile = 0;
+    int chains = 0, chain_min_rows = 0;
+    hipStream_t chain_stream = nullptr;
+    hipEvent_t chain_ev[3] = {nullptr, nullptr, nullptr};
+    int64_t chain_calls = 0;
     bool prof = false;
     std::vector<std::pair<hipEvent_t, hipEvent_t>> ev_pool;
     size_t ev_used = 0;
diff --git a/sgpt_amd/csrc/ctx.hip b/sgpt_amd/csrc/ctx.hip
--- a/sgpt_amd/csrc/ctx.hip
+++ b/sgpt_amd/csrc/ctx.hip
@@ -60,6 +60,8 @@
     if (c->ws6) (void)hipFree(c->ws6);
     if (c->range_flag) (void)hipFree(c->range_flag);
     for (auto& e : c->ev_pool) { (void)hipEventDestroy(e.first); (void)hipEventDestroy(e.second); }
+    for (hipEvent_t e : c->chain_ev) if (e) (void)hipEventDestroy(e);
+    if (c->chain_stream) (void)hipStreamDestroy(c->chain_stream);
     delete c;
 }
 
@@ -131,6 +133,14 @@
     c->no_qpath = policy == 2 ? 1 : 0;
     return old;
 }
+int32_t sgpt_ctx_set_encode_chains(sgpt_ctx* c, int32_t n, int32_t min_rows) {
+    if (!c || n < 0 || n > 2 || min_rows < 0) return -1;
+    const int old = c->chains;
+    c->chains = n;
+    c->chain_min_rows = min_rows;
+    return old;
+}
+int64_t sgpt_ctx_encode_chain_calls(const sgpt_ctx* c) { return c ? c->chain_calls : 0; }
 int32_t sgpt_ctx_set_query_tile(sgpt_ctx* c, int32_t k) {
     if (!c || k < 0 || k > 7) return -1;
     const int old = c->qtile;
diff --git a/sgpt_amd/csrc/encode.hip b/sgpt_amd/csrc/encode.hip
--- a/sgpt_amd/csrc/encode.hip
+++ b/sgpt_amd/csrc/encode.hip
@@ -1,4 +1,5 @@
 #include "host.h"
+#include "encode_split.h"
 
 namespace {
 
@@ -16,6 +17,9 @@
     void* gu;
     void* a8; float* sa;
     long att_lo;
+    long ldvt;
+    long row0; int b0;
+    hipEvent_t half_ev;
 };
 
 GemmArgs proj(const Fwd& f, const void* A, long lda, const void* W, int N, int K, void* out, long ldo, const float* bias,
@@ -35,7 +39,7 @@
     gemm(f.c, f.dt, EPI_STORE, f.dt, qk, f.s);
     if (p_ln1 == 2) split_w(v, (const bf16_t*)W3 + (size_t)n_qk * 3 * g.K, g.K);
     else v.W = (const bf16_t*)g.W + (size_t)n_qk * g.K;
-    v.N = n_v; v.out = f.vt; v.ldo = f.T; v.bias = g.bias ? g.bias + n_qk : nullptr;
+    v.N = n_v; v.out = f.vt; v.ldo = f.ldvt; v.bias = g.bias ? g.bias + n_qk : nullptr;
     gemm(f.c, f.dt, EPI_VT, f.dt, v, f.s);
 }
 
@@ -48,8 +52,12 @@
     at.scale = d.attn_scale * pow2f(2 * k_qkv);
     at.max_alloc_len = f.max_alloc; at.ctx = f.ctx; at.ldo = dq; at.alibi = f.m->alibi;
     at.q = f.qkv; at.kv_group = d.n_heads / d.n_kv_heads;
-    if (f.vt) { at.k = (bf16_t*)f.qkv + dq; at.v = f.vt; at.ldq = dq + f.d_kv; at.ldvt = f.T; }
+    if (f.vt) { at.k = (bf16_t*)f.qkv + dq; at.v = f.vt; at.ldq = dq + f.d_kv; at.ldvt = f.ldvt; }
     else { at.k = (float*)f.qkv + dq; at.v = (float*)f.qkv + dq + f.d_kv; at.ldq = dq + 2 * f.d_kv; }
+    if (f.row0) {
+        at.ctx = (bf16_t*)f.ctx - f.row0 * dq; at.q = (bf16_t*)f.qkv - f.row0 * at.ldq; at.k = (const bf16_t*)at.q + dq;
+        at.v = (bf16_t*)f.vt - f.row0;
+    }
     return at;
 }
 
@@ -77,7 +85,7 @@
     const int dm = d.d_model, ffn = d.d_ffn, T = f.T, dt = f.dt;
     GemmArgs q = proj(f, f.a, dm, l.w_qkv, 3 * dm, dm, f.qkv, 2 * dm, l.b_qkv);
     if (gemm_qkv_one_launch(T, 2 * dm, f.c->force256 != 0)) {
-        q.n_split = 2 * dm; q.out2 = f.vt; q.ldo2 = T;
+        q.n_split = 2 * dm; q.out2 = f.vt; q.ldo2 = f.ldvt;
         gemm(f.c, dt, EPI_QKV, dt, q, f.s);
     } else proj_qk_vt(f, q, 2 * dm, dm);
     launch_attn_bf16(attn_bidir(f, l), f.s);
@@ -213,7 +221,7 @@
         if (f.qpath || ((p_ln1 == 0 || p_ln1 == 2) && gemm_qkv_one_launch(T, 2 * dm, c->force256 != 0)) ||
             (p_ln1 == 0 && !p_att && l.b_qkv == nullptr && gemm_qkv_bulk(T, 3 * dm, dm, 2 * dm, c->force256 != 0))) {
             if (p_ln1 == 2) split_w(q.g, l.w_qkv3, dm);
-            q.g.n_split = 2 * dm; q.g.out2 = f.vt; q.g.ldo2 = T;
+            q.g.n_split = 2 * dm; q.g.out2 = f.vt; q.g.ldo2 = f.ldvt;
             if ((st = launch16(f, EPI_QKV, dt, q, "QKV projection")) != SGPT_OK) return st;
         } else {
             proj_qk_vt(f, q.g, 2 * dm, dm, l.w_qkv3, p_ln1);
@@ -234,6 +242,7 @@
         q.g.in_mul = pow2f(k_qkv);
         if ((st = launch16(f, EPI_BIAS_RESID, SGPT_F32, q, "out-projection")) != SGPT_OK) return st;
     }
+    if (f.half_ev) HIPC(c, hipEventRecord(f.half_ev, s));
     {
         QGemmArgs q{};
         q.g = proj(f, f.a, lda2, l.w_fc, ffn, dm, f.h, ldh, l.b_fc);
@@ -333,6 +342,7 @@
     if (f.mlp8) { f.a8 = base + o_a8; f.sa = (float*)(base + o_sa); }
     if (lp) *lp = (float*)(base + o_lp);
     f.att_lo = (long)(qkv_bytes / 2);
+    f.ldvt = T;
     return SGPT_OK;
 }
 
@@ -350,12 +360,70 @@
     return SGPT_OK;
 }
 
+
+#ifndef SGPT_CHAINS_DEFAULT
+#define SGPT_CHAINS_DEFAULT 2
+#endif
+constexpr int CHAINS_DEFAULT = SGPT_CHAINS_DEFAULT;
+constexpr int CHAINS_AUTO_ROWS = 131072;
+#ifndef SGPT_CHAIN_PHASE
+#define SGPT_CHAIN_PHASE 1
+#endif
+constexpr int CHAIN_PHASE = SGPT_CHAIN_PHASE;
+
+EncodeSplit chain_cut(const Fwd& f, BlockFn block, const int32_t* seq_off_host, bool pooled_only) {
+    sgpt_model* m = f.m; sgpt_ctx* c = f.c;
+    const EncodeSplit none{0, 0};
+    const int mode = c->chains ? c->chains : CHAINS_DEFAULT;
+    const int dm = m->d.d_model, ffn = m->d.d_ffn;
+    if (mode != 2 || !seq_off_host || !pooled_only || block != block_16) return none;
+    if (f.qpath || f.fp8 || f.mlp8 || f.split || m->calibrating || m->probing) return none;
+    if (f.T < (c->chain_min_rows > 0 ? c->chain_min_rows : CHAINS_AUTO_ROWS) || f.T % ENCODE_SPLIT_TILE != 0) return none;
+    const EncodeSplit cut = encode_split_point(seq_off_host, f.B, f.T);
+    if (cut.row == 0) return none;
+    const bool f256 = c->force256 != 0;
+    for (int rows : {cut.row, f.T - cut.row})
+        if (!gemm_bulk_256(rows, 2 * dm, dm, EPI_STORE, f256) || !gemm_bulk_256(rows, dm, dm, EPI_VT, f256) ||
+            !gemm_bulk_256(rows, dm, dm, EPI_BIAS_RESID, f256) || !gemm_bulk_256(rows, ffn, dm, EPI_BIAS_GELU, f256) ||
+            !gemm_bulk_256(rows, dm, ffn, EPI_BIAS_RESID, f256))
+            return none;
+    hipStreamCaptureStatus cap = hipStreamCaptureStatusNone;
+    if (hipStreamIsCapturing(f.s, &cap) != hipSuccess) { (void)hipGetLastError(); return none; }
+    return cap == hipStreamCaptureStatusNone ? cut : none;
+}
+
+sgpt_status chain_init(sgpt_ctx* c) {
+    if (!c->chain_stream) HIPC(c, hipStreamCreateWithFlags(&c->chain_stream, hipStreamNonBlocking));
+    for (hipEvent_t& e : c->chain_ev)
+        if (!e) HIPC(c, hipEventCreateWithFlags(&e, hipEventDisableTiming));
+    return SGPT_OK;
+}
+
+Fwd chain_of(const Fwd& f, int row0, int rows, int b0, int nb, hipStream_t s) {
+    const size_t dm = f.m->d.d_model, ffn = f.m->d.d_ffn, r = row0;
+    Fwd h = f;
+    h.s = s; h.row0 = row0; h.b0 = b0; h.T = rows; h.B = nb;
+    h.pos += r; h.seq_off += b0; h.seq_len += b0;
+    h.x += r * dm;
+    h.a = (bf16_t*)f.a + r * dm; h.ctx = (bf16_t*)f.ctx + r * dm; h.qkv = (bf16_t*)f.qkv + r * 2 * dm; h.vt = (bf16_t*)f.vt + r;
+    h.h = (bf16_t*)f.h + r * ffn;
+    return h;
+}
+
+sgpt_status zero_cut_overread(const Fwd& f, int r) {
+    const size_t dm = f.m->d.d_model;
+    HIPC(f.c, hipMemsetAsync((bf16_t*)f.qkv + (size_t)r * 2 * dm, 0, (size_t)256 * 2 * dm * 2, f.s));
+    HIPC(f.c, hipMemset2DAsync((bf16_t*)f.vt + r, (size_t)f.ldvt * 2, 0, SLACK * 2, dm, f.s));
+    return SGPT_OK;
+}
+
 }
 
 static sgpt_status encode_impl(sgpt_model* m, const int32_t* ids, const int32_t* pos, const int32_t* seq_off,
                                const int32_t* seq_len, const int32_t* pad_left, int32_t B, int32_t T, int32_t max_alloc,
                                int32_t pool_mode, int32_t n_layers_run, int32_t apply_final_ln, int32_t normalize,
-                               float* out, float* hidden_out, float* layer_out, float* layer_mean, void* stream) {
+                               float* out, float* hidden_out, float* layer_out, float* layer_mean, void* stream,
+                               const int32_t* seq_off_host = nullptr) {
     if (!m) return SGPT_ERR_INVALID;
     sgpt_ctx* c = m->ctx;
     const Family& F = family(m->d.arch);
@@ -373,10 +441,43 @@
         launch_lnf_pool(x, m->lnf_g, m->lnf_b, seq_off, seq_len, pad_left, B, dm, m->d.ln_eps, final_ln, pool_mode, normalize, m->pool_w,
                         m->pool_w_n, dst, s, range_flag, F.norm_kind);
     };
-    launch_embed(ids, pos, m->wte, m->wpe, x, T, dm, m->d.vocab, m->d.max_pos, s);
-    if (F.post_ln && f.vt) launch_layernorm_writeback(x, m->emb_ln_g, m->emb_ln_b, f.a, dt, T, dm, m->d.ln_eps, f.range_flag, s);
-    else if (m->emb_ln_g) launch_layernorm(x, m->emb_ln_g, m->emb_ln_b, x, SGPT_F32, T, dm, m->d.ln_eps, s);
+    auto embed = [&](const Fwd& g) {
+        launch_embed(ids + g.row0, g.pos, m->wte, m->wpe, g.x, g.T, dm, m->d.vocab, m->d.max_pos, g.s);
+        if (F.post_ln && g.vt) launch_layernorm_writeback(g.x, m->emb_ln_g, m->emb_ln_b, g.a, dt, g.T, dm, m->d.ln_eps, g.range_flag, g.s);
+        else if (m->emb_ln_g) launch_layernorm(g.x, m->emb_ln_g, m->emb_ln_b, g.x, SGPT_F32, g.T, dm, m->d.ln_eps, g.s);
+    };
     const BlockFn block = pick_block(f);
+    const EncodeSplit cut = chain_cut(f, block, seq_off_host, out && !hidden_out && !layer_out && !layer_mean);
+    if (cut.row) {
+        if ((st = chain_init(c)) != SGPT_OK || (st = zero_cut_overread(f, cut.row)) != SGPT_OK) return st;
+        hipStream_t sb = c->chain_stream;
+        const Fwd fa = chain_of(f, 0, cut.row, 0, cut.seq, s), fb = chain_of(f, cut.row, T - cut.row, cut.seq, B - cut.seq, sb);
+        HIPC(c, hipEventRecord(c->chain_ev[0], s));
+        HIPC(c, hipStreamWaitEvent(sb, c->chain_ev[0], 0));
+        embed(fa);
+        if (CHAIN_PHASE == 0 || n_layers_run == 0) embed(fb);
+        for (int li = 0; li < n_layers_run; ++li) {
+            Fwd a = fa;
+            if (li == 0 && CHAIN_PHASE == 1) a.half_ev = c->chain_ev[1];
+            if ((st = block(a, m->L[li], li)) != SGPT_OK) return st;
+            if (li == 0 && CHAIN_PHASE != 0) {
+                if (CHAIN_PHASE == 2) HIPC(c, hipEventRecord(c->chain_ev[1], s));
+                HIPC(c, hipStreamWaitEvent(sb, c->chain_ev[1], 0));
+                embed(fb);
+            }
+            if ((st = block(fb, m->L[li], li)) != SGPT_OK) return st;
+        }
+        int* rf = m->d.compute_dtype == SGPT_F16 ? (int*)m->range_dev : nullptr;
+        for (const Fwd* g : {&fa, &fb})
+            launch_lnf_pool(x, m->lnf_g, m->lnf_b, g->seq_off, g->seq_len, pad_left ? pad_left + g->b0 : nullptr, g->B, dm, m->d.ln_eps,
+                            apply_final_ln, pool_mode, normalize, m->pool_w, m->pool_w_n, out + (size_t)g->b0 * dm, g->s, rf, F.norm_kind);
+        HIPC(c, hipEventRecord(c->chain_ev[2], sb));
+        HIPC(c, hipStreamWaitEvent(s, c->chain_ev[2], 0));
+        c->chain_calls++;
+        HIPC(c, hipGetLastError());
+        return SGPT_OK;
+    }
+    embed(f);
     for (int li = 0; li < n_layers_run; ++li) {
         LayerW l = m->L[li];
         if (layer_out) pool(0, layer_out + (size_t)li * B * dm, nullptr);
@@ -409,6 +510,14 @@
                         float* out, float* hidden_out, void* stream) {
     return encode_impl(m, ids, pos, seq_off, seq_len, pad_left, B, T, max_alloc, pool_mode, n_layers_run,
                        apply_final_ln, normalize, out, hidden_out, nullptr, nullptr, stream);
+}
+
+sgpt_status sgpt_encode_host_layout(sgpt_model* m, const int32_t* ids, const int32_t* pos, const int32_t* seq_off,
+                                    const int32_t* seq_len, const int32_t* pad_left, int32_t B, int32_t T, int32_t max_alloc,
+                                    int32_t pool_mode, int32_t n_layers_run, int32_t apply_final_ln, int32_t normalize,
+                                    float* out, float* hidden_out, const int32_t* seq_off_host, void* stream) {
+    return encode_impl(m, ids, pos, seq_off, seq_len, pad_left, B, T, max_alloc, pool_mode, n_layers_run,
+                       apply_final_ln, normalize, out, hidden_out, nullptr, nullptr, stream, seq_off_host);
 }
 
 sgpt_status sgpt_encode_layers(sgpt_model* m, const int32_t* ids, const int32_t* pos, const int32_t* seq_off,
diff --git a/sgpt_amd/csrc/encode_split.h b/sgpt_amd/csrc/encode_split.h
--- /dev/null
+++ b/sgpt_amd/csrc/encode_split.h
@@ -0,0 +1,21 @@
+#pragma once
+#include <cstdint>
+
+constexpr int ENCODE_SPLIT_TILE = 256;
+
+struct EncodeSplit { int32_t row, seq; };
+
+inline EncodeSplit encode_split_point(const int32_t* seq_off, int32_t B, int32_t T) {
+    EncodeSplit best{0, 0};
+    if (!seq_off || B < 2 || T <= 0 || seq_off[0] != 0) return best;
+    int64_t best_dist = -1;
+    for (int32_t b = 1; b <= B; ++b)
+        if (seq_off[b] <= seq_off[b - 1] || seq_off[b] > T) return EncodeSplit{0, 0};
+    for (int32_t b = 1; b < B; ++b) {
+        const int64_t o = seq_off[b];
+        if (o % ENCODE_SPLIT_TILE != 0 || 3 * o < T || 3 * o > 2 * (int64_t)T) continue;
+        const int64_t dist = 2 * o > T ? 2 * o - T : T - 2 * o;
+        if (best_dist < 0 || dist < best_dist) { best_dist = dist; best = EncodeSplit{(int32_t)o, b}; }
+    }
+    return best;
+}
diff --git a/sgpt_amd/csrc/gemm.hip b/sgpt_amd/csrc/gemm.hip
--- a/sgpt_amd/csrc/gemm.hip
+++ b/sgpt_amd/csrc/gemm.hip
@@ -902,6 +902,13 @@
     return M % 256 == 0 && N % 256 == 0 && n_split % 256 == 0 && n_split < N && K % 64 == 0 && K >= 128 &&
            (long)(M / 256) * (n_split / 256) > SGPT_FEW_TILES;
 }
+bool gemm_bulk_256(int M, int N, int K, int epi, bool force256) {
+    if (exp_env("SGPT_GEMM128") != nullptr) return false;
+    const bool small_tiles = exp_env("SGPT_NO_SMALL_TILE") == nullptr;
+    const long few_limit = epi_is_gelu(epi) ? 255 : SGPT_FEW_TILES;
+    const bool few = small_tiles && !force256 && (long)(M / 256) * (N / 256) <= few_limit;
+    return M > 0 && M % 256 == 0 && N % 256 == 0 && K % 64 == 0 && K >= 128 && !few;
+}
 bool gemm_score_tail_foldable(int M, long N, int K) {
     if (exp_env("SGPT_GEMM128") != nullptr) return false;
     return score_tail_foldable_shape(M, N, K);
diff --git a/sgpt_amd/model.py b/sgpt_amd/model.py
--- a/sgpt_amd/model.py
+++ b/sgpt_amd/model.py
@@ -44,6 +44,7 @@
     max_pos: int = 0
     arena: Optional[torch.Tensor] = None
     n_real: int = 0
+    off_host: Optional[np.ndarray] = None
 
 
 def _flatten(seqs, total: int) -> np.ndarray:
@@ -458,13 +459,14 @@
         dev = into.arena if into is not None else torch.empty(n_int, dtype=torch.int32, device=self.device)
         dev.copy_(host[:n_int], non_blocking=True)
         self._staging.release(slot)
+        off_host = np.ascontiguousarray(lay["off"], dtype=np.int32)
         if into is not None:
-            into.n_tokens, into.max_pos, into.n_real = lay["n_tokens"], lay["max_pos"], lay["n_real"]
+            into.n_tokens, into.max_pos, into.n_real, into.off_host = lay["n_tokens"], lay["max_pos"], lay["n_real"], off_host
             return into
         o = 2 * T
         return PackedBatch(dev[:T], dev[T:o], dev[o: o + B + 1], dev[o + B + 1: o + 2 * B + 1],
                            dev[o + 2 * B + 1: o + 3 * B + 1], B, T, lay["max_alloc"], lay["n_tokens"], lay["max_pos"],
-                           arena=dev, n_real=lay["n_real"])
+                           arena=dev, n_real=lay["n_real"], off_host=off_host)
 
     def encode_packed(self, pb: PackedBatch, mode: str = "weightedmean", normalize: bool = False,
                       layer_idx: int = -1, out: Optional[torch.Tensor] = None,
@@ -481,10 +483,11 @@
         if out is None:
             out = torch.empty((pb.B, d), dtype=torch.float32, device=self.device)
         hidden = torch.empty((pb.T_pad, d), dtype=torch.float32, device=self.device) if return_hidden else None
-        st = self.ctx.lib.sgpt_encode(self.handle, _p(pb.ids), _p(pb.pos), _p(pb.seq_off), _p(pb.seq_len),
-                                      _p(pb.pad_left), pb.B, pb.T_pad, pb.max_alloc, POOL_MODES[mode], n_run,
-                                      final_ln, 1 if normalize else 0, _p(out), _p(hidden),
-                                      _stream_ptr(self.device))
+        off_host = pb.off_host.ctypes.data if pb.off_host is not None and pb.off_host.size == pb.B + 1 else None
+        st = self.ctx.lib.sgpt_encode_host_layout(self.handle, _p(pb.ids), _p(pb.pos), _p(pb.seq_off), _p(pb.seq_len),
+                                                  _p(pb.pad_left), pb.B, pb.T_pad, pb.max_alloc, POOL_MODES[mode], n_run,
+                                                  final_ln, 1 if normalize else 0, _p(out), _p(hidden), off_host,
+                                                  _stream_ptr(self.device))
         _lib.check(self.ctx.handle, st, "sgpt_encode")
         return (out, hidden) if return_hidden else out
 
diff --git a/sgpt_amd/runtime.py b/sgpt_amd/runtime.py
--- a/sgpt_amd/runtime.py
+++ b/sgpt_amd/runtime.py
@@ -164,6 +164,15 @@
 
     def set_query_tile(self, k: int) -> int:
         return int(self.lib.sgpt_ctx_set_query_tile(self.handle, int(k)))
+
+    def set_encode_chains(self, n: int, min_rows: int = 0) -> int:
+        old = int(self.lib.sgpt_ctx_set_encode_chains(self.handle, int(n), int(min_rows)))
+        if old < 0:
+            raise ValueError("set_encode_chains: n in (0, 1, 2), min_rows >= 0")
+        return old
+
+    def encode_chain_calls(self) -> int:
+        return int(self.lib.sgpt_ctx_encode_chain_calls(self.handle))
 
     def reserve(self, encode_bytes: int = 0, score_bytes: int = 0) -> None:
         self._chk(self.lib.sgpt_ctx_reserve(self.handle, encode_bytes, score_bytes), "sgpt_ctx_reserve")
```

Measured after the change: 38790, median of 6. +2.2%, better.
